# Tzq2doc/distributed_learning_simulator

Measured on AMD Instinct MI355X. Metric: FL rounds/sec (FedAvg, 100 clients, ResNet-18, CIFAR-10-shaped), higher is better.
Workload: dtype fp32; 1 GPU; fedavg_resnet18; model=ResNet18, algo=fed_avg, clients=100, local_epochs=5, global_batch=6400, per_client_batch=64, parallelism=client-dp1, backend=hip

## Files before the change

csrc/bindings.cpp:

```cpp
#include <pybind11/pybind11.h>

#include <algorithm>
#include <optional>
#include <stdexcept>
#include <string>
#include <vector>

#include "dls.h"

namespace py = pybind11;
typedef uintptr_t ptr;

template <typename T>
static T* P(ptr p) {
  return reinterpret_cast<T*>(p);
}
static hipStream_t S(ptr s) { return reinterpret_cast<hipStream_t>(s); }

extern "C" const char* dls_src_hash();

class Args {
 public:
  struct Ptr {
    uintptr_t v;
// ... 55 lines not shown
  if (!a.on()) return e;
  e.theta = a.p("theta"); e.mom = a.p("mom"); e.split = a.p("split");
  e.th_cs = a.l("th_cs"); e.sp_cs = a.l("sp_cs"); e.sp_lo = a.l("sp_lo");
  e.lr = a.p("lr"); e.active = a.p("active"); e.first = a.p("first");
  e.wd = a.f("wd"); e.momentum = a.f("momentum"); e.dampening = a.f("dampening"); e.nesterov = a.i("nesterov");
  a.finish();
  return e;
}

PYBIND11_MODULE(_dls_hip, m) {
  m.doc() = "gfx950 kernels for the MI355X-native cohort FL simulator";
  m.def("src_hash", []() { return std::string(dls_src_hash()); });
  m.def("set_native_option", [](const std::string& name, int value) {
    if (!set_native_option(name.c_str(), value)) throw std::invalid_argument("unknown native option " + name);
  });

  m.def("conv_nt", [](py::kwargs kw) {
    Args a(kw, "conv_nt");
    ConvNTParams p{};
    p.x = a.p("x"); p.w = a.p("w"); p.y = a.p("y"); p.bias = a.p("bias", 0); p.b_cs = a.l("b_cs", 0);
    p.acc = a.p("acc", 0); p.gate = a.p("gate", 0); p.x_cs = a.l("x_cs"); p.y_cs = a.l("y_cs"); p.w_cs = a.l("w_cs");
    p.B = a.i("B"); p.H = a.i("H"); p.W = a.i("W"); p.C = a.i("C"); p.OH = a.i("OH"); p.OW = a.i("OW");
    p.KH = a.i("KH"); p.KW = a.i("KW"); p.stride = a.i("stride"); p.pad = a.i("pad"); p.dil = a.i("dil");
    p.M = a.i("M"); p.N = a.i("N"); p.R = a.i("R"); p.rep = a.i("rep"); p.relu = a.i("relu", 0);
    p.b_kmajor = a.i("b_kmajor", 0); p.f32 = a.i("f32"); p.ldx = a.i("ldx", 0); p.ldy = a.i("ldy", 0);
    p.stats = a.p("stats", 0); p.stats_valid = a.p("stats_valid", 0); p.drop_seeds = a.p("drop_seeds", 0);
    p.drop_p = a.f("drop_p", 0.f); p.out_scale = a.f("out_scale", 0.f); p.wsplit = a.p("wsplit", 0);
    p.ws_cs = a.l("ws_cs", 0); p.ws_plane = a.l("ws_plane", 0); p.x_lo = a.l("x_lo", 0);
    p.yp = a.p("yp", 0); p.yp_cs = a.l("yp_cs", 0); p.yp_lo = a.l("yp_lo", 0);
    const int K = a.i("K"), variant = a.i("variant");
    const hipStream_t s = a.p("s");
    a.finish();
    if (p.stats && p.stats_valid && native_option(g_opt_halo_skip, "DLS_SKIP_INVALID", 1)) {
      p.skip_valid = p.stats_valid;
      p.skip_mul = p.OH * p.OW;
    }
    conv_nt(p, K, variant, s);
  });
  m.def("conv_dgrad", [](py::kwargs kw) {
    Args a(kw, "conv_dgrad");
    const auto dy = a.p("dy"), w = a.p("w"), acc = a.p("acc", 0), wsplit = a.p("wsplit", 0);
    const auto dx = a.p("dx"), wt_buf = a.p("wt_buf", 0), acc_mask = a.p("acc_mask", 0), s = a.p("s");
    const int K = a.i("K"), rep = a.i("rep"), B = a.i("B"), OH = a.i("OH"), OW = a.i("OW"), Co = a.i("Co");
    const int H = a.i("H"), W = a.i("W"), Ci = a.i("Ci"), KH = a.i("KH"), KW = a.i("KW"), stride = a.i("stride");
    const int pad = a.i("pad"), variant = a.i("variant"), f32 = a.i("f32"), ld_dy = a.i("ld_dy", 0);
    const int acc_compact = a.i("acc_compact", 0), wt_ready = a.i("wt_ready", 0);
    const long w_cs = a.l("w_cs"), dy_cs = a.l("dy_cs", 0), ws_cs = a.l("ws_cs", 0), ws_plane = a.l("ws_plane", 0);
    const long x_lo = a.l("x_lo", 0);
    Args b = a.sub("bnb");
    BNBwdPartials bnb{};
    if (b.on()) {
      bnb.part = b.p("part"); bnb.x = b.p("x"); bnb.xld = b.l("xld", 0); bnb.y = b.p("y", 0);
      bnb.mask = b.p("mask", 0); bnb.mean = b.p("mean"); bnb.rstd = b.p("rstd"); bnb.valid = b.p("valid", 0);
      b.finish();
    }
    a.finish();
    conv_dgrad(dy, w, dx, acc, w_cs, K, rep, B, OH, OW, Co, H, W, Ci, KH, KW, stride, pad, variant, f32, s, ld_dy,
               dy_cs, wsplit, ws_cs, ws_plane, x_lo, acc_compact, bnb.part ? &bnb : nullptr, wt_buf, acc_mask, wt_ready);
  });
  m.def("wt_planes", [](ptr wsplit, long ws_cs, long ws_plane, ptr wt, int Kw, int Co, int Ci, ptr s) {
    wt_planes(P<const bf16_t>(wsplit), ws_cs, ws_plane, P<bf16_t>(wt), Kw, Co, Ci, S(s));
  });
  m.def("conv_gl_wanted", &conv_gl_wanted);
  m.def("conv_gl_fwd", [](ptr x, ptr w, ptr y, ptr bias, long x_cs, long y_cs, long w_cs, long b_cs, int K, int rep,
                          int B, int H, int W, int C, int OH, int OW, int KH, int KW, int stride, int pad, int N,
                          int relu, ptr s) {
    conv_gl_fwd(P<const bf16_t>(x), P<const bf16_t>(w), P<bf16_t>(y), P<const bf16_t>(bias), x_cs, y_cs, w_cs, b_cs,
                K, rep, B, H, W, C, OH, OW, KH, KW, stride, pad, N, relu, S(s));
  });
  m.def("conv_weight_flip_t", [](ptr w, ptr wt, long w_cs, int Kw, int Co, int KH, int KW, int Ci, ptr s) {
    conv_weight_flip_t(P<const bf16_t>(w), P<bf16_t>(wt), w_cs, Kw, Co, KH, KW, Ci, S(s));
  });
  m.def("conv_gl_dgrad", [](ptr dy, ptr wt, ptr dx, ptr acc, int K, int rep, int B, int OH, int OW, int Co, int H, int W,
                            int Ci, int KH, int KW, int stride, int pad, ptr s) {
    conv_gl_dgrad(P<const bf16_t>(dy), P<const bf16_t>(wt), P<bf16_t>(dx), P<const bf16_t>(acc), K, rep, B, OH, OW, Co, H, W, Ci, KH, KW,
                  stride, pad, S(s));
  });
  m.def("conv_nt_num_variants", &conv_nt_num_variants);
  m.def("conv_nt_default_variant", &conv_nt_default_variant);
  m.def("conv_tn_f32_bn_bwd_ok", &conv_tn_f32_bn_bwd_ok);
  m.def("conv_tn", [](py::kwargs kw) {
    Args a(kw, "conv_tn");
    ConvTNParams p{};
    p.dy = a.p("dy"); p.x = a.p("x"); p.dw = a.p("dw");
    p.dy_cs = a.l("dy_cs"); p.x_cs = a.l("x_cs"); p.dw_cs = a.l("dw_cs");
    p.B = a.i("B"); p.H = a.i("H"); p.W = a.i("W"); p.C = a.i("C"); p.OH = a.i("OH"); p.OW = a.i("OW");
    p.KH = a.i("KH"); p.KW = a.i("KW"); p.stride = a.i("stride"); p.pad = a.i("pad");
    p.M = a.i("M"); p.Co = a.i("Co"); p.R = a.i("R"); p.splitk = 1; p.m_per_split = p.M;
    p.f32 = a.i("f32"); p.ldy = a.i("ldy", 0); p.ldx = a.i("ldx", 0);
    p.part = a.p("part", 0); p.dy_lo = a.l("dy_lo", 0); p.x_lo = a.l("x_lo", 0);
    p.sgd = sgd_arg(a.sub("sgd"));
    p.bnb_x = a.p("bnb_x", 0); p.bnb_mask = a.p("bnb_mask", 0);
    p.bnb_coef = a.p("bnb_coef", 0); p.bnb_valid = a.p("bnb_valid", 0);
    const int K = a.i("K"), variant = a.i("variant");
    const hipStream_t s = a.p("s");
    a.finish();
    conv_tn(p, K, variant, s);
  });
  m.def("conv_tn_splitk", &conv_tn_splitk, py::arg("K"), py::arg("Co"), py::arg("R"), py::arg("M"), py::arg("C"),
        py::arg("variant"), py::arg("f32"), py::arg("ldy") = 0, py::arg("ldx") = 0, py::arg("planes") = 0);
  m.def("conv_tn_pl_num_variants", &conv_tn_pl_num_variants);
  m.def("conv_tn_pl_set_variant", &conv_tn_pl_set_variant);
  m.def("conv_tn_pl_variant", &conv_tn_pl_variant);
  m.def("conv_tn_num_variants", &conv_tn_num_variants);
  m.def("conv_nt_f32_num_variants", &conv_nt_f32_num_variants);
  m.def("conv_nt_pl_num_variants", &conv_nt_pl_num_variants);
// ... 74 lines not shown
    const auto gamma = a.p("gamma"), dgamma = a.p("dgamma", 0), dbeta = a.p("dbeta", 0), ws = a.p("ws");
    const auto s = a.p("s");
    const long g_cs = a.l("g_cs"), dg_cs = a.l("dg_cs", 0);
    a.finish();
    return dense_dgrad_bn(p, gamma, g_cs, dgamma, dbeta, dg_cs, ws, s);
  });
  m.def("halo_wgrad_supported", &halo_wgrad_supported);
  m.def("halo_wgrad_part_floats", &halo_wgrad_part_floats);
  m.def("halo_wgrad", [](py::kwargs kw) {
    Args a(kw, "halo_wgrad");
    HaloWgradParams p{};
    p.sgd = sgd_arg(a.sub("sgd"));
    Args b = a.sub("bnb");
    if (b.on()) {
      p.bb_x = b.p("bb_x"); p.bb_mask = b.p("bb_mask", 0); p.bb_coef = b.p("bb_coef");
      p.bb_valid = b.p("bb_valid", 0); p.bb_dxp = b.p("bb_dxp");
      b.finish();
    }
    p.dy = a.p("dy"); p.dy_cs = a.l("dy_cs"); p.dy_lo = a.l("dy_lo", 0); p.ldy = a.i("ldy");
    p.x = a.p("x"); p.x_cs = a.l("x_cs"); p.x_lo = a.l("x_lo", 0); p.ldx = a.i("ldx");
    p.coef = a.p("coef", 0); p.relu = a.i("relu", 0); p.x_valid = a.p("x_valid", 0);
    p.valid_img = a.p("valid_img", 0); p.dw = a.p("dw"); p.dw_cs = a.l("dw_cs"); p.part = a.p("part", 0);
    p.K = a.i("K"); p.B = a.i("B"); p.H = a.i("H"); p.W = a.i("W"); p.C = a.i("C"); p.N = a.i("N");
    const int xm = a.i("xm"), dm = a.i("dm");
    const hipStream_t s = a.p("s");
    a.finish();
    return halo_wgrad(p, xm, dm, s);
  });
  m.def("conv_halo_bn_dense_supported", &conv_halo_bn_dense_supported);
  m.def("conv_halo_bn_dense_fwd", [](py::kwargs kw) {
    Args a(kw, "conv_halo_bn_dense_fwd");
    const auto x = a.p("x"), coef = a.p("coef"), valid_rows = a.p("valid_rows", 0), wsplit = a.p("wsplit");
    const auto y = a.p("y"), stats = a.p("stats", 0), stats_valid = a.p("stats_valid", 0), s = a.p("s");
    const auto ny = a.p("ny", 0), mask = a.p("mask", 0);
    const long x_cs = a.l("x_cs"), ws_cs = a.l("ws_cs"), ws_plane = a.l("ws_plane"), y_cs = a.l("y_cs");
    const long ny_cs = a.l("ny_cs", 0);
    const int ldx = a.i("ldx"), creal = a.i("creal"), relu = a.i("relu", 0), rep = a.i("rep"), ldy = a.i("ldy");
    const int K = a.i("K"), B = a.i("B"), H = a.i("H"), W = a.i("W"), C = a.i("C"), N = a.i("N"), ldny = a.i("ldny", 0);
    a.finish();
    return conv_halo_bn_dense_fwd(x, x_cs, ldx, creal, coef, relu, valid_rows, wsplit, ws_cs, ws_plane, rep, y, y_cs,
                                  ldy, K, B, H, W, C, N, stats, stats_valid, ny, ny_cs, ldny, mask, s);
  });
  m.def("bn_bwd", [](py::kwargs kw) {
    Args a(kw, "bn_bwd");
    const auto dy = a.p("dy"), x = a.p("x"), y = a.p("y", 0), mean = a.p("mean", 0);
    const auto rstd = a.p("rstd", 0), gamma = a.p("gamma", 0), valid_rows = a.p("valid_rows", 0);
    const auto dx = a.p("dx", 0), dpre = a.p("dpre", 0), dgamma = a.p("dgamma", 0);
    const auto dbeta = a.p("dbeta", 0), ws = a.p("ws"), relu_mask = a.p("relu_mask", 0), s = a.p("s");
    const auto dxp = a.p("dxp", 0), pre_part = a.p("pre_part", 0), coef_ext = a.p("coef_ext", 0);
    const long g_cs = a.l("g_cs", 0), dg_cs = a.l("dg_cs", 0);
    const int K = a.i("K"), R = a.i("R"), C = a.i("C"), relu = a.i("relu", 0), f32 = a.i("f32");
    const int ldx = a.i("ldx", 0), acc_dx = a.i("acc_dx", 0), dx_f32 = a.i("dx_f32", 1);
    const int pre_nparts = a.i("pre_nparts", 0), stage = a.i("stage", 0);
    a.finish();
    bn_bwd(dy, x, y, mean, rstd, gamma, valid_rows, g_cs, K, R, C, relu, dx, dpre, dgamma, dbeta, dg_cs, ws, relu_mask,
           f32, s, ldx, acc_dx, dxp, dx_f32, pre_part, pre_nparts, coef_ext, stage);
  });
  m.def("ln_fwd", [](ptr x, ptr gamma, ptr beta, ptr y, ptr mean, ptr rstd, long g_cs, int K, long rpc, int C,
                     float eps, int rep, int f32, ptr s, ptr yp) {
    ln_fwd(P<const void>(x), P<const void>(gamma), P<const void>(beta), P<void>(y), P<float>(mean), P<float>(rstd),
           g_cs, K, rpc, C, eps, rep, f32, S(s), P<bf16_t>(yp));
  });
  m.def("ln_bwd", [](ptr dy, ptr x, ptr mean, ptr rstd, ptr gamma, long g_cs, int K, long rpc, int C, ptr dx,
                     ptr dgamma, ptr dbeta, long dg_cs, int f32, ptr s, ptr ws) {
    ln_bwd(P<const void>(dy), P<const void>(x), P<const float>(mean), P<const float>(rstd), P<const void>(gamma), g_cs,
           K, rpc, C, P<void>(dx), P<float>(dgamma), P<float>(dbeta), dg_cs, P<float>(ws), f32, S(s));
  });
  m.def("ln_workspace_floats", &ln_workspace_floats);
  m.def("gn_shape_ok", &gn_shape_ok);
  m.def("gn_workspace_floats", &gn_workspace_floats);
  m.def("gn_fwd", [](ptr x, ptr res, ptr gamma, ptr beta, ptr y, ptr yp, ptr mean, ptr rstd, ptr valid, long g_cs,
                     int rep, int K, int B, int HW, int C, int G, float eps, int relu, int f32, ptr s) {
    gn_fwd(P<const void>(x), P<const void>(res), P<const void>(gamma), P<const void>(beta), P<void>(y), P<bf16_t>(yp),
           P<float>(mean), P<float>(rstd), P<const int>(valid), g_cs, rep, K, B, HW, C, G, eps, relu, f32, S(s));
  });
  m.def("gn_bwd", [](ptr dy, ptr x, ptr y, ptr mean, ptr rstd, ptr gamma, ptr valid, long g_cs, int rep, int K, int B,
                     int HW, int C, int G, int relu, ptr dx, ptr dres, ptr dgamma, ptr dbeta, long dg_cs, ptr ws,
                     int f32, ptr s) {
    gn_bwd(P<const void>(dy), P<const void>(x), P<const void>(y), P<const float>(mean), P<const float>(rstd),
           P<const void>(gamma), P<const int>(valid), g_cs, rep, K, B, HW, C, G, relu, P<void>(dx), P<void>(dres),
           P<float>(dgamma), P<float>(dbeta), dg_cs, P<float>(ws), f32, S(s));
  });
  m.def("col_sum_workspace_floats", &col_sum_workspace_floats);
  m.def("col_sum", [](ptr x, ptr out, long out_cs, int K, long rows, int C, int f32, ptr s, ptr ws) {
    col_sum(P<const void>(x), P<float>(out), out_cs, K, rows, C, f32, S(s), P<float>(ws));
  });

  m.def("pool_fwd", [](ptr x, ptr y, ptr idx, int K, int B, int H, int W, int C, int OH, int OW, int k, int stride,
                       int pad, int mode, int f32, ptr s) {
    pool_fwd(P<const void>(x), P<void>(y), P<int>(idx), K, B, H, W, C, OH, OW, k, stride, pad, mode, f32, S(s));
  });
  m.def("pool_bwd", [](ptr dy, ptr idx, ptr dx, int K, int B, int H, int W, int C, int OH, int OW, int k, int stride,
                       int pad, int mode, int f32, ptr s) {
    pool_bwd(P<const void>(dy), P<const int>(idx), P<void>(dx), K, B, H, W, C, OH, OW, k, stride, pad, mode, f32, S(s));
  });
  m.def("gap_fwd", [](ptr x, ptr y, int KB, int HW, int C, int f32, ptr s) {
    gap_fwd(P<const void>(x), P<void>(y), KB, HW, C, f32, S(s));
  });
  m.def("gap_bwd", [](ptr dy, ptr dx, int KB, int HW, int C, int f32, ptr s) {
    gap_bwd(P<const void>(dy), P<void>(dx), KB, HW, C, f32, S(s));
  });
  m.def("ce_fwd_bwd", [](ptr logits, ptr labels, ptr valid, ptr loss, ptr correct, ptr dlogits, int K, int B, int NC,
                         int f32, ptr s, ptr rowbuf) {
    ce_fwd_bwd(P<const void>(logits), P<const int>(labels), P<const int>(valid), P<float>(loss), P<float>(correct),
               P<void>(dlogits), K, B, NC, f32, S(s), P<float>(rowbuf));
  });
  m.def("relu_bwd", [](ptr dy, ptr y, ptr dx, long n, int f32, ptr s) {
    relu_bwd(P<const void>(dy), P<const void>(y), P<void>(dx), n, f32, S(s));
  });

// ... 227 lines not shown
```

csrc/conv_f32.hip:

```cpp
#include "dls.h"
#include "gemm_common.h"
#include "epilogue_f32.h"

#include <numeric>

namespace {

template <int V>
struct FV {
  float v[V];
};

template <int V>
__device__ __forceinline__ void fzero(FV<V>& f) {
#pragma unroll
  for (int i = 0; i < V; ++i) f.v[i] = 0.f;
}

template <int V>
__device__ __forceinline__ void fload(FV<V>& f, const float* p) {
  load_vec<V>(p, f.v);
}

template <int V>
// ... 231 lines not shown
#pragma unroll
      for (int j = 0; j < TN; ++j) {
        if constexpr (!BKM) {
          const int r = wn0 + j * 32 + (lane & 31);
          const int off = (buf * B_ROWS + r) * B_COLS + swz<BK>(r, ks * 16 + 8 * h);
          bh[j] = *reinterpret_cast<const bf16x8*>(Bs + off);
          bl[j] = *reinterpret_cast<const bf16x8*>(Bs + B_PLANE + off);
        } else {
          const int col = wn0 + j * 32 + 16 * (g & 1) + 4 * pp;
          const int o0 = (buf * B_ROWS + ks * 16 + 8 * h + q) * B_COLS + col;
          const int o1 = o0 + 4 * B_COLS;
          bh[j] = tr_frag(Bs + o0, Bs + o1);
          bl[j] = tr_frag(Bs + B_PLANE + o0, Bs + B_PLANE + o1);
        }
      }
#pragma unroll
      for (int i = 0; i < TM; ++i)
#pragma unroll
        for (int j = 0; j < TN; ++j) {
          acc[i][j] = __builtin_amdgcn_mfma_f32_32x32x16_bf16(al[i], bh[j], acc[i][j], 0, 0, 0);
          acc[i][j] = __builtin_amdgcn_mfma_f32_32x32x16_bf16(ah[i], bl[j], acc[i][j], 0, 0, 0);
          acc[i][j] = __builtin_amdgcn_mfma_f32_32x32x16_bf16(ah[i], bh[j], acc[i][j], 0, 0, 0);
        }
    }
  };

  if constexpr (NBUF == 1) {
    load();
    store(0);
    __syncthreads();
    for (int kt = 0; kt < nk; ++kt) {
      if (kt + 1 < nk) load();
      compute(0);
      if (kt + 1 < nk) {
        __syncthreads();
        store(0);
        __syncthreads();
      }
    }
  } else {
    load();
    store(0);
    __syncthreads();
    int buf = 0;
    for (int kt = 0; kt < nk; ++kt) {
      if (kt + 1 < nk) load();
      compute(buf);
      if (kt + 1 < nk) store(buf ^ 1);
      __syncthreads();
      buf ^= 1;
    }
  }

  nt_f32_epilogue<TM, TN, WM * WN, -1, false>(p, acc, smem, client, m0, n0, wm0, wn0, wid, lane);
}

template <int BM, int BN, int BK, int WM, int WN, int NBUF, int VSET, int MINW = 1>
bool launch_nt_f32_cfg(const ConvNTParams& p, int K, int va, int vb, bool bkm, hipStream_t s) {
  const int grid = K * cdiv(p.M, BM) * cdiv(p.N, BN);
  if (p.wsplit && va == 8 && vb == 8) {
    if (bkm)
      hipLaunchKernelGGL((conv_nt_f32_kernel<BM, BN, BK, WM, WN, 8, 8, true, NBUF, MINW, true>), dim3(grid),
                         dim3(WM * WN * 64), 0, s, p);
    else
      hipLaunchKernelGGL((conv_nt_f32_kernel<BM, BN, BK, WM, WN, 8, 8, false, NBUF, MINW, true>), dim3(grid),
                         dim3(WM * WN * 64), 0, s, p);
    return true;
  }
#define NTF_CASE(A, B)                                                                                       \
  if (va == A && vb == B) {                                                                                  \
    if (bkm)                                                                                                 \
      hipLaunchKernelGGL((conv_nt_f32_kernel<BM, BN, BK, WM, WN, A, B, true, NBUF, MINW>), dim3(grid),             \
                         dim3(WM * WN * 64), 0, s, p);                                                       \
    else                                                                                                     \
      hipLaunchKernelGGL((conv_nt_f32_kernel<BM, BN, BK, WM, WN, A, B, false, NBUF, MINW>), dim3(grid),            \
                         dim3(WM * WN * 64), 0, s, p);                                                       \
    return true;                                                                                             \
  }
  NTF_CASE(8, 8)
  if constexpr (VSET >= 1) { NTF_CASE(4, 4) NTF_CASE(8, 4) NTF_CASE(4, 8) }
  if constexpr (VSET >= 2) { NTF_CASE(8, 1) NTF_CASE(4, 1) NTF_CASE(1, 8) NTF_CASE(1, 4) NTF_CASE(1, 1) }
#undef NTF_CASE
  return false;
}

bool launch_nt_f32_variant(int v, const ConvNTParams& p, int K, int va, int vb, bool bkm, hipStream_t s) {
  switch (v) {
    case 0: return launch_nt_f32_cfg<128, 128, 32, 2, 2, 2, 1>(p, K, va, vb, bkm, s);
    case 1: return launch_nt_f32_cfg<128, 128, 32, 2, 2, 1, 0>(p, K, va, vb, bkm, s);
    case 2: return launch_nt_f32_cfg<256, 128, 32, 4, 2, 1, 0>(p, K, va, vb, bkm, s);
    case 3: return launch_nt_f32_cfg<64, 64, 32, 2, 2, 2, 2>(p, K, va, vb, bkm, s);
    case 4: return launch_nt_f32_cfg<128, 64, 32, 4, 1, 2, 1>(p, K, va, vb, bkm, s);
    case 5: return launch_nt_f32_cfg<128, 128, 64, 2, 2, 1, 0>(p, K, va, vb, bkm, s);
    case 6: return launch_nt_f32_cfg<256, 64, 32, 4, 1, 1, 0>(p, K, va, vb, bkm, s);
    case 7: return launch_nt_f32_cfg<64, 64, 32, 2, 2, 1, 1>(p, K, va, vb, bkm, s);
    case 8: return launch_nt_f32_cfg<128, 128, 32, 2, 2, 1, 0, 3>(p, K, va, vb, bkm, s);
    case 9: return launch_nt_f32_cfg<256, 64, 32, 4, 1, 1, 0, 3>(p, K, va, vb, bkm, s);
    case 10: return launch_nt_f32_cfg<256, 32, 32, 4, 1, 1, 1>(p, K, va, vb, bkm, s);
    default: return false;
  }
}

int vw(int c) { return (c % 8 == 0) ? 8 : (c % 4 == 0) ? 4 : 1; }


template <int BMc, int BNr, int BKT, int WM, int WN, int VA, int VB, int NBUF, bool BNB = false>
__global__ void __launch_bounds__(WM* WN * 64) conv_tn_f32_kernel(ConvTNParams p) {
// ... 317 lines not shown
  (void)K;
  const TnTile t = kTnF32Tiles[variant];
  const long tiles = (long)32 * cdiv(Co, t.bm) * cdiv(R, t.bn);
  splitk = 1;
  const int target = 1024;
  if (tiles < target) {
    splitk = (int)((target + tiles - 1) / tiles);
    splitk = min(splitk, max(1, M / (4 * TN_BKT_MAX)));
  }
  mps = cdiv(M, splitk);
  mps = ((mps + TN_BKT_MAX - 1) / TN_BKT_MAX) * TN_BKT_MAX;
  splitk = cdiv(M, mps);
}

}

int conv_nt_f32_num_variants() { return 11; }

void conv_nt_f32(const ConvNTParams& p, int K, int variant, hipStream_t s) {
  if (p.x_lo != 0) {
    if (conv_nt_pl_variant() < 0 && conv_halo(p, K, s)) return;
    if (!conv_nt_pl(p, K, conv_nt_pl_variant(), s)) {
      fprintf(stderr, "conv_nt_f32: pre-split operands in an unsupported shape (C %d, ldx %d, N %d, R %d)\n", p.C,
              p.ldx, p.N, p.R);
      abort();
    }
    return;
  }
  const bool bkm = p.b_kmajor != 0;
  const long xb = (long)p.B * p.H * p.W * p.ldx * 4;
  const long wb = (bkm ? (long)p.C * p.wKH * p.wKW * p.N : (long)p.N * p.R) * 4;
  if (p.dil != 1) {
    fprintf(stderr, "conv_nt_f32: input dilation is not supported\n");
    abort();
  }
  if (xb >= (long)OOB_OFF || wb >= (long)OOB_OFF || (p.wsplit && (p.ws_plane + wb / 4) * 2 >= (long)OOB_OFF)) {
    fprintf(stderr, "conv_nt_f32: per-client operand window over 2 GiB (x %ld B, w %ld B)\n", xb, wb);
    abort();
  }
  const int va = vw(std::gcd(p.C, p.ldx));
  int vb = bkm ? vw(p.N) : vw(p.R);
  if (variant < 0) {
    variant = p.N <= 64 ? 9 : 1;
    if (p.N <= 32) variant = 10;
    if (p.N > 64 && p.KH * p.KW == 1) variant = 8;
  }
  const bool v88 = va == 8 && vb == 8;
  const bool v84 = (va == 8 || va == 4) && (vb == 8 || vb == 4);
  if (!v88) {
    if (!v84 && variant != 3) variant = 3;
    if (v84 && !(variant == 0 || variant == 3 || variant == 4 || variant == 7 || variant == 10))
      variant = p.N <= 64 ? 4 : 0;
  }
  if (!launch_nt_f32_variant(variant, p, K, va, vb, bkm, s)) fprintf(stderr, "conv_nt_f32: bad variant %d\n", variant);
  if (p.yp) {
    if (p.yp_cs != 2 * p.y_cs || p.yp_lo != p.y_cs || p.ldy != p.N || p.out_s != 1) {
      fprintf(stderr, "conv_nt_f32: output planes need contiguous per-client rows\n");
      abort();
    }
    split_rows(reinterpret_cast<const float*>(p.y), p.yp, K, (long)p.M * p.N, p.y_cs, s);
  }
}

int conv_tn_f32_num_variants() { return kTnF32Variants; }

void conv_tn_f32(ConvTNParams p, int K, int variant, hipStream_t s) {
  if (p.sgd.theta && p.dy_lo == 0) {
    fprintf(stderr, "conv_tn_f32: the SGD epilogue needs pre-split operands\n");
    abort();
  }
  if (p.dy_lo != 0) {
    if (!conv_tn_pl(p, K, variant, s)) {
      fprintf(stderr, "conv_tn_f32: pre-split operands in an unsupported shape (C %d, Co %d)\n", p.C, p.Co);
      abort();
    }
    return;
  }
  const long dyb = (long)p.M * (p.ldy ? p.ldy : p.Co) * 4, xb = (long)p.B * p.H * p.W * (p.ldx ? p.ldx : p.C) * 4;
  if (dyb >= (long)OOB_OFF || xb >= (long)OOB_OFF) {
    fprintf(stderr, "conv_tn_f32: per-client operand window over 2 GiB (dy %ld B, x %ld B)\n", dyb, xb);
    abort();
  }
  const int va = vw(std::gcd(p.Co, p.ldy));
  const int vb = vw(std::gcd(p.C, p.ldx));
  variant = resolve_tn_f32_variant(variant, K, p.Co, p.R, va, vb);
  if (p.bnb_coef && !(p.bnb_x && p.ldy == p.Co && p.dy_cs == (long)p.M * p.Co && va == 8 && vb == 8 &&
                      tn_f32_bnb_variant(variant))) {
    fprintf(stderr, "conv_tn_f32: the BN-backward loader does not serve this launch (Co %d, C %d, variant %d)\n",
            p.Co, p.C, variant);
    abort();
  }
  tn_f32_split(K, p.Co, p.R, p.M, variant, p.splitk, p.m_per_split);
  const TnTile t = kTnF32Tiles[variant];
  const long tiles = (long)K * cdiv(p.Co, t.bm) * cdiv(p.R, t.bn);
  const int grid = (int)(tiles * p.splitk);
  if (!launch_tn_f32_variant(variant, p, va, vb, grid, s)) fprintf(stderr, "conv_tn_f32: bad variant %d\n", variant);
  if (p.splitk > 1 && p.part != nullptr) tn_fold(p.part, p.dw, p.dw_cs, K, p.splitk, (long)p.Co * p.R, s);
}

bool conv_tn_f32_bn_bwd_ok(int K, int Co, int R, int gco, int gc, int variant) {
  const int va = vw(gco), vb = vw(gc);
  return va == 8 && vb == 8 && tn_f32_bnb_variant(resolve_tn_f32_variant(variant, K, Co, R, va, vb));
}

int conv_tn_f32_splitk(int K, int Co, int R, int M, int gco, int gc, int variant) {
  int splitk, mps;
// ... 5 lines not shown
```

csrc/conv_nt.hip:

```cpp
#include "dls.h"
#include "gemm_common.h"

#include <numeric>

namespace {

template <int BM, int BN, int BK, int WM, int WN, int VA, int VB, bool BKM, int DEPTH>
__global__ void __launch_bounds__(WM* WN * 64) conv_nt_kernel(ConvNTParams p) {
  constexpr int T = WM * WN * 64;
  constexpr int TM = BM / (WM * 32);
  constexpr int TN = BN / (WN * 32);
  constexpr int LDA = BK + 8;
  constexpr int KCA = BK / VA, RPA = T / KCA, PA = BM / RPA;
  constexpr int KCB = BK / VB, RPB = T / KCB, PB = BN / RPB;
  constexpr int CCB = BN / VB, RPK = T / CCB, PK = BK / RPK;
  constexpr int LDBK = BN + 32;
  constexpr int NB = BKM ? PK : PB;
  static_assert(PA >= 1 && NB >= 1, "tile too small for thread count");
  static_assert(TM >= 1 && TN >= 1, "wave tile");
  constexpr int NBUF = DEPTH == 0 ? 1 : 2;
  constexpr int B_ROWS = BKM ? BK : BN, B_COLS = BKM ? LDBK : LDA;
  constexpr int A_BYTES = NBUF * BM * LDA * 2, B_BYTES = NBUF * B_ROWS * B_COLS * 2;
  constexpr int SW = TN * 32 + 8;
  constexpr int EPI_BYTES = WM * WN * 32 * SW * 2;
// ... 335 lines not shown
  if (p.wKH == 0) {
    p.pad_w = p.pad;
    p.wKH = p.KH;
    p.wKW = p.KW;
    p.kh_off = p.KH - 1;
    p.kw_off = p.KW - 1;
    p.kh_step = p.kw_step = 1;
  }
  if (p.out_s == 0) p.out_s = 1;
  if (p.ldx == 0) p.ldx = p.C;
  if (p.ldy == 0) p.ldy = p.N;
  p.fd_ohw = make_fastdiv((uint32_t)(p.OH * p.OW));
  p.fd_ow = make_fastdiv((uint32_t)p.OW);
  p.fd_kwc = make_fastdiv((uint32_t)(p.KW * p.C));
  p.fd_c = make_fastdiv((uint32_t)p.C);
  if (p.f32) {
    conv_nt_f32(p, K, variant, s);
    return;
  }
  if (p.stats) {
    fprintf(stderr, "conv_nt: epilogue statistics need the fp32 kernels\n");
    abort();
  }
  const bool bkm = p.b_kmajor != 0;
  int va = vec_width(std::gcd(p.C, p.ldx));
  int vb = bkm ? vec_width(p.N) : vec_width(p.R);
  if (va == 1 && vb == 4) vb = 1;
  if (variant < 0) {
    variant = conv_nt_default_variant(p.M, p.N, p.R, p.b_kmajor);
    (void)K;
  }
  const bool w84 = (va == 8 || va == 4) && (vb == 8 || vb == 4);
  if (w84 && !(va == 8 && vb == 8) && !(variant == 0 || variant == 10 || variant == 13 || variant == 6 ||
                                        variant == 7 || variant == 18)) {
    variant = (p.N <= 64) ? 13 : (bkm ? 10 : 0);
  } else if (!w84 && !(variant == 6 || variant == 7 || variant == 18)) {
    variant = (p.N <= 64) ? 7 : 6;
  }
  if (!launch_variant(variant, p, K, va, vb, bkm, s)) fprintf(stderr, "conv_nt: bad variant %d\n", variant);
}

void wt_planes(const bf16_t* wsplit, long ws_cs, long ws_plane, bf16_t* wt, int Kw, int Co, int Ci, hipStream_t s) {
  hipLaunchKernelGGL(wt_planes_kernel, dim3(Kw * 2 * 9, Co / 32, Ci / 32), dim3(256), 0, s, wsplit, ws_cs, ws_plane, wt,
                     Co, Ci);
}

void conv_dgrad(const bf16_t* dy, const bf16_t* w, bf16_t* dx, const bf16_t* acc, long w_cs, int K, int rep, int B, int OH, int OW,
                int Co, int H, int W, int Ci, int KH, int KW, int stride, int pad, int variant, int f32, hipStream_t s,
                int ld_dy, long dy_cs, const bf16_t* wsplit, long ws_cs, long ws_plane, long x_lo, int acc_compact,
                const BNBwdPartials* bnb, bf16_t* wt_buf, const uint8_t* acc_mask, int wt_ready) {
  ConvNTParams p{};
  p.acc_mask = acc_mask;
  if (bnb) {
    if (!f32 || stride != 1 || Ci % 4 != 0 || (bnb->mask && Ci % 8 != 0) || (bnb->xld && bnb->xld % 4 != 0)) {
      fprintf(stderr, "conv_dgrad: BN-backward partials need an fp32 stride-1 dgrad with Ci %% 4 == 0\n");
      abort();
    }
    p.bnb = bnb->part;
    p.bnb_x = bnb->x;
    p.bnb_xld = bnb->xld ? bnb->xld : Ci;
    p.bnb_y = bnb->y;
    p.bnb_mask = bnb->mask;
    p.bnb_mean = bnb->mean;
    p.bnb_rstd = bnb->rstd;
    p.bnb_valid = bnb->valid;
    if (stride == 1 && bnb->valid && native_option(g_opt_halo_skip, "DLS_SKIP_INVALID", 1)) {
      p.skip_valid = bnb->valid;
      p.skip_mul = 1;
    }
  }
  p.x_lo = x_lo;
  p.wsplit = wsplit;
  p.ws_cs = ws_cs;
  p.ws_plane = ws_plane;
  p.f32 = f32;
  p.ldx = ld_dy;
  p.x = dy;
  p.w = w;
  p.y = dx;
  p.bias = nullptr;
  p.acc = acc;
  p.x_cs = dy_cs ? dy_cs : (long)B * OH * OW * (ld_dy ? ld_dy : Co);
  p.y_cs = (long)B * H * W * Ci;
  p.w_cs = w_cs;
  p.b_cs = 0;
  p.B = B;
  p.H = OH;
  p.W = OW;
  p.C = Co;
  p.N = Ci;
  p.rep = rep;
  p.relu = 0;
  p.b_kmajor = 1;
  p.wKH = KH;
  p.wKW = KW;
  p.dil = 1;
  p.stride = 1;
  if (stride == 1) {
    p.OH = H;
    p.OW = W;
    p.KH = KH;
    p.KW = KW;
    p.pad = KH - 1 - pad;
    p.pad_w = KW - 1 - pad;
    p.kh_off = KH - 1;
    p.kw_off = KW - 1;
    p.kh_step = p.kw_step = 1;
    p.out_s = 1;
    p.M = B * H * W;
    p.R = KH * KW * Co;
    if (variant < 0 && !f32 && Ci <= 64 && vec_width(Ci) == 8 && vec_width(Co) == 8) variant = 14;
    if (wt_buf && f32 && x_lo != 0 && wsplit && KH == 3 && KW == 3 && pad == 1 && Co % 32 == 0 && Ci % 32 == 0) {
      const int Kw = K / rep;
      if (!wt_ready)
        hipLaunchKernelGGL(wt_planes_kernel, dim3(Kw * 2 * 9, Co / 32, Ci / 32), dim3(256), 0, s, wsplit, ws_cs,
                           ws_plane, wt_buf, Co, Ci);
      p.b_kmajor = 0;
      p.wsplit = wt_buf;
      p.ws_cs = 2L * 9 * Ci * Co;
      p.ws_plane = 9L * Ci * Co;
      p.w = wt_buf;
      p.w_cs = p.ws_cs;
    }
    conv_nt(p, K, variant, s);
    return;
  }
  for (int ph = 0; ph < stride; ++ph) {
    const int Hc = (H - ph + stride - 1) / stride;
    if (Hc <= 0) continue;
    const int kh0 = (ph + pad) % stride;
    const int nkh = kh0 < KH ? (KH - kh0 + stride - 1) / stride : 0;
    const int dh = (ph + pad - kh0) / stride;
    for (int pw = 0; pw < stride; ++pw) {
      const int Wc = (W - pw + stride - 1) / stride;
      if (Wc <= 0) continue;
      const int kw0 = (pw + pad) % stride;
      const int nkw = kw0 < KW ? (KW - kw0 + stride - 1) / stride : 0;
      const int dw = (pw + pad - kw0) / stride;
      ConvNTParams q = p;
      q.OH = Hc;
      q.OW = Wc;
      q.M = B * Hc * Wc;
      if (acc_compact) {
        q.acc = (ph == 0 && pw == 0) ? acc : nullptr;
        q.acc_compact = 1;
        q.acc_cs = (long)B * Hc * Wc * Ci;
      }
      q.out_s = stride;
      q.out_ph = ph;
      q.out_pw = pw;
      q.out_H = H;
      q.out_W = W;
      if (nkh == 0 || nkw == 0) {
        q.KH = q.KW = 1;
        q.R = 0;
        q.pad = q.pad_w = 0;
        q.kh_off = q.kw_off = 0;
        q.kh_step = q.kw_step = 1;
      } else {
        q.KH = nkh;
        q.KW = nkw;
        q.pad = nkh - 1 - dh;
        q.pad_w = nkw - 1 - dw;
        q.kh_off = kh0 + stride * (nkh - 1);
        q.kw_off = kw0 + stride * (nkw - 1);
        q.kh_step = q.kw_step = stride;
        q.R = nkh * nkw * Co;
      }
      conv_nt(q, K, variant, s);
    }
  }
}
```

csrc/conv_pl.hip:

```cpp
#include "dls.h"
#include "epilogue_f32.h"
#include "sgd_epi.h"
#include "gemm_common.h"

#include <algorithm>
#include <cstdlib>

namespace {

constexpr int PK = 32;

typedef __attribute__((address_space(3))) void lds_void;

__device__ __forceinline__ void dma16(__amdgpu_buffer_rsrc_t r, unsigned char* lds, uint32_t off) {
  __builtin_amdgcn_raw_ptr_buffer_load_lds(r, (lds_void*)lds, 16, off, 0, 0, 0);
}

template <int N>
__device__ __forceinline__ void wait_vm() {
  static_assert(N >= 0 && N < 64, "vmcnt range");
  __builtin_amdgcn_s_waitcnt((N & 15) | ((N >> 4) << 14) | (7 << 4) | (15 << 8));
}

template <int BM, int BN, int WM, int WN, bool BKM, int NST, int MINW, bool ILV, int PKT, bool PIX = false>
// ... 193 lines not shown
      for (int i = 0; i < TM; ++i) {
        if (PIX && !on[i]) continue;
#pragma unroll
        for (int j = 0; j < TN; ++j) {
          acc[i][j] = __builtin_amdgcn_mfma_f32_32x32x16_bf16(al[i], bh[j], acc[i][j], 0, 0, 0);
          acc[i][j] = __builtin_amdgcn_mfma_f32_32x32x16_bf16(ah[i], bl[j], acc[i][j], 0, 0, 0);
          acc[i][j] = __builtin_amdgcn_mfma_f32_32x32x16_bf16(ah[i], bh[j], acc[i][j], 0, 0, 0);
          if constexpr (ILV) {
            static_assert(!ILV || !PIX, "the interleaved DMAs must issue with every triple");
            const int tri = (ks * TM + i) * TN + j;
#pragma unroll
            for (int n = 0; n < G; ++n)
              if ((n * NTRI) / G == tri) {
                piece(n, nb);
                __builtin_amdgcn_sched_group_barrier(0x008, 3, 0);
                __builtin_amdgcn_sched_group_barrier(0x020, 1, 0);
              }
          }
        }
      }
    }
    if constexpr (PIX) {
      c_kc += PKT;
      if (c_kc == p.C) {
        c_kc = 0;
        if (++c_kw > tb.w1) {
          c_kw = tb.w0;
          ++c_kh;
        }
      }
    }
  };

  const int nk = PIX ? (tb.h1 - tb.h0 + 1) * (tb.w1 - tb.w0 + 1) * (p.C / PKT) : p.R / PKT;
#pragma unroll
  for (int st = 0; st < NST - 1; ++st) {
    prep(st < nk);
#pragma unroll
    for (int n = 0; n < G; ++n) piece(n, st);
  }
  for (int kt = 0; kt < nk; ++kt) {
    wait_vm<G*(NST - 2)>();
    __builtin_amdgcn_s_barrier();
    const int nb = (kt + NST - 1) % NST;
    prep(kt + NST - 1 < nk);
    if constexpr (!ILV) {
#pragma unroll
      for (int n = 0; n < G; ++n) piece(n, nb);
    }
    compute(kt % NST, nb);
  }
  wait_vm<0>();

  nt_f32_epilogue<TM, TN, NW, -1, true, PIX>(p, acc, smem, client, m0, n0, wm0, wn0, wid, lane);
}

template <int BM, int BN, int WM, int WN, int NST, bool ILV = false, int PKT = 32, int MINW = 1, bool PIX = false>
void launch_pl(const ConvNTParams& p, int K, bool bkm, hipStream_t s) {
  const int grid = K * cdiv(p.M, BM) * cdiv(p.N, BN);
  if (bkm)
    hipLaunchKernelGGL((conv_nt_pl_kernel<BM, BN, WM, WN, true, NST, MINW, ILV, PKT, PIX>), dim3(grid),
                       dim3(WM * WN * 64), 0, s, p);
  else
    hipLaunchKernelGGL((conv_nt_pl_kernel<BM, BN, WM, WN, false, NST, MINW, ILV, PKT, PIX>), dim3(grid),
                       dim3(WM * WN * 64), 0, s, p);
}

}

static int g_pl_variant = -1;
int conv_nt_pl_variant() { return g_pl_variant; }
void conv_nt_pl_set_variant(int v) { g_pl_variant = v; }

int conv_nt_pl_num_variants() { return 8; }

bool conv_nt_pl_supported(const ConvNTParams& p) {
  return p.x_lo != 0 && p.wsplit != nullptr && p.dil == 1 && p.C % PK == 0 && p.ldx % 8 == 0 &&
         p.N % 8 == 0 && (p.R == p.KH * p.KW * p.C || p.R == 0);
}

static int pl_min_wg() {
  return native_option(g_opt_pl_min_wg, "DLS_PL_MIN_WG", 192);
}

int conv_nt_pl_default_variant(const ConvNTParams& p, int K) {
  if (p.N <= 64) return 2;
  if (p.N >= 512) return (long)K * cdiv(p.M, 256) * cdiv(p.N, 256) < pl_min_wg() ? 1 : 3;
  if (p.M >= (1 << 17)) {
    if (p.N >= 256) return 3;
    if (p.KH * p.KW > 1) return 4;
  }
  return 1;
}

static bool pix_ok(const ConvNTParams& p, int variant) {
  return native_option(g_opt_conv_pix, "DLS_CONV_PIX", 1) != 0 && variant == 3 && p.stride == 1 &&
         p.OH * p.OW <= 64 && p.KH * p.KW > 1 && (p.pad > 0 || p.pad_w > 0) && p.out_s <= 1 && !p.acc_compact &&
         !(p.drop_p > 0.f) && p.M == p.B * p.OH * p.OW;
}

bool conv_nt_pl(const ConvNTParams& p0, int K, int variant, hipStream_t s) {
  if (!conv_nt_pl_supported(p0)) return false;
  const long ab = (p0.x_lo + (long)p0.B * p0.H * p0.W * p0.ldx) * 2;
  const long wb = (p0.ws_plane + (p0.b_kmajor ? (long)p0.C * p0.wKH * p0.wKW * p0.N : (long)p0.N * p0.R)) * 2;
  if (ab >= (long)OOB_OFF || wb >= (long)OOB_OFF) return false;
  if (variant < 0) variant = conv_nt_pl_default_variant(p0, K);
  const bool bkm = p0.b_kmajor != 0;
// ... 438 lines not shown
```

csrc/dls.h:

```cpp
#pragma once
#include <hip/hip_runtime.h>
#include <stdint.h>

typedef uint16_t bf16_t;

constexpr int kOptUnset = -1000000;
extern int g_opt_attn_mfma, g_opt_conv_gl, g_opt_pl_min_wg;
extern int g_opt_halo_wgrad_unroll;
extern int g_opt_halo_skip;
extern int g_opt_conv_pix;
int native_option(int& slot, const char* env, int dflt);
bool set_native_option(const char* name, int value);

struct FastDiv {
  uint32_t d, mul, shift;
};

static inline FastDiv make_fastdiv(uint32_t d) {
  FastDiv f;
  f.d = d;
  uint32_t s = 0;
  while ((1u << s) < d) ++s;
  f.shift = s;
  f.mul = (uint32_t)((((uint64_t)1 << 32) * (((uint64_t)1 << s) - d)) / d + 1);
  return f;
}

__device__ __forceinline__ uint32_t fdiv(uint32_t n, const FastDiv& f) {
  return (__umulhi(n, f.mul) + n) >> f.shift;
}

struct ConvNTParams {
  const bf16_t* x;
  const bf16_t* w;
  bf16_t* y;
  const bf16_t* bias;
  const bf16_t* acc;
  long acc_cs;
  int acc_compact;
  const uint8_t* acc_mask;
  const bf16_t* gate;
  long x_cs, y_cs, w_cs, b_cs;
  int B, H, W, C;
  int OH, OW, KH, KW, stride, pad, dil;
  int pad_w;
  int M, N, R;
  int rep;
  int relu;
  int b_kmajor;
  int wKH, wKW, kh_off, kh_step, kw_off, kw_step;
  int out_s, out_ph, out_pw, out_H, out_W;
  FastDiv fd_ohw, fd_ow, fd_kwc, fd_c;
  int f32;
  int ldx, ldy;
  float* stats;
  const int* stats_valid;
  const uint32_t* drop_seeds;
  float drop_p;
  float out_scale;
  const bf16_t* wsplit;
  long ws_cs, ws_plane;
  long x_lo;
  float* bnb;
  const float* bnb_x;
  long bnb_xld;
  const float* bnb_y;
  const uint8_t* bnb_mask;
  const float* bnb_mean;
  const float* bnb_rstd;
  const int* bnb_valid;
  const float* bn_x;
  long bn_x_cs;
  const float* bn_coef;
  int bn_relu;
  const int* bn_valid;
  bf16_t* bn_yp;
  uint8_t* bn_mask;
  int bn_c;
  float* bn_y;
  long bn_y_cs;
  int bn_ldy;
  const int* skip_valid;
  int skip_mul;
  bf16_t* yp;
  long yp_cs, yp_lo;
  int pix;
  FastDiv fd_pb;
};

struct BNBwdPartials {
  float* part;
  const float* x;
  long xld;
  const float* y;
  const uint8_t* mask;
  const float* mean;
  const float* rstd;
  const int* valid;
};

struct DenseWgradParams {
  const float* dy;
  long dy_cs;
  int ldy;
  const float* y;
  long y_cs;
  float* dw;
  long dw_cs;
  float* part;
  int K, B, H, W, C, N, nchunks, G;
  const float* bn_sc;
  int ldy_x;
  const int* valid_rows;
};

struct DenseDgradParams {
  const float* dy;
  long dy_cs;
  int ldy;
  const float* w;
  long w_cs;
  int rep;
  const float* x;
  float* dx;
  long x_cs;
  int ldx;
  const uint8_t* mask;
  const float* y;
  const float* bn_sc;
  const float* mean;
  const float* rstd;
  const int* valid_rows;
  const float* coef;
  float* part;
  int K, B, H, W, C, N, G, nchunks;
};

struct SgdEpi {
  float* theta;
  float* mom;
  bf16_t* split;
  long th_cs, sp_cs, sp_lo;
  const float* lr;
  const uint8_t* active;
  const uint8_t* first;
  float wd, momentum, dampening;
  int nesterov;
};

struct HaloWgradParams {
  const void* dy;
// ... 108 lines not shown
bool conv_halo_bn_fwd(const float* x, long x_cs, const float* coef, int relu, const int* valid_rows,
                      const bf16_t* wsplit, long ws_cs, long ws_plane, int rep, float* y, long y_cs, int K, int B,
                      int H, int W, int C, int N, float* stats, const int* stats_valid, hipStream_t s,
                      bf16_t* yp = nullptr, uint8_t* mask = nullptr);
bool conv_halo_bn_dense_supported(int B, int H, int W, int C, int N);
bool conv_halo_bn_dense_fwd(const float* x, long x_cs, int ldx, int creal, const float* coef, int relu,
                            const int* valid_rows, const bf16_t* wsplit, long ws_cs, long ws_plane, int rep, float* y,
                            long y_cs, int ldy, int K, int B, int H, int W, int C, int N, float* stats,
                            const int* stats_valid, float* ny, long ny_cs, int ldny, uint8_t* mask, hipStream_t s);
bool dense_dgrad_supported(int B, int H, int W, int C, int N);
long dense_dgrad_ws_floats(int K, int B, int H, int C);
bool dense_dgrad_bn(DenseDgradParams p, const float* gamma, long g_cs, float* dgamma, float* dbeta, long dg_cs,
                    float* ws, hipStream_t s);
void bn_bwd_coef_parts(const float* part, int nparts, const float* gamma, long g_cs, const int* valid_rows,
                       const float* mean, const float* rstd, int K, int R, int C, float* coef, float* dgamma,
                       float* dbeta, long dg_cs, hipStream_t s);
bool dense_wgrad_supported(int B, int H, int W, int C, int N);
long dense_wgrad_part_floats(int K, int B, int H, int W, int C);
bool dense_wgrad(const float* dy, long dy_cs, int ldy, const float* y, long y_cs, float* dw, long dw_cs, float* part,
                 int K, int B, int H, int W, int C, int N, hipStream_t s, const float* bn_sc = nullptr,
                 int ldy_x = 0, const int* valid_rows = nullptr);
void conv_halo_set_mode(int m);
void conv_halo_set_variant(int v);
bool conv_tn_pl_supported(const ConvTNParams& p);
bool conv_tn_pl(ConvTNParams p, int K, int variant, hipStream_t s);
int conv_tn_pl_num_variants();
int conv_tn_pl_variant();
void conv_tn_pl_set_variant(int v);
int conv_tn_pl_splitk(int K, int Co, int R, int M, int variant);
void tn_fold(const float* part, float* dw, long dw_cs, int K, int splitk, long CoR, hipStream_t s,
             const SgdEpi* sgd = nullptr);
int conv_tn_f32_num_variants();
int conv_tn_f32_splitk(int K, int Co, int R, int M, int gco, int gc, int variant);
bool conv_tn_f32_bn_bwd_ok(int K, int Co, int R, int gco, int gc, int variant);

long bn_workspace_floats(int K, long R, int C);
void bn_fwd(const void* x, const void* gamma, const void* beta, const void* res, void* y, float* mean, float* rstd,
            const int* valid_rows, long g_cs, int K, int R, int C, int relu, float eps, int rep, float* ws,
            uint8_t* relu_mask, int f32, hipStream_t s,
            int ldx = 0, const float* pre_part = nullptr,
            int pre_nparts = 0, bf16_t* yp = nullptr,
            int y_f32 = 1, float* coef_out = nullptr, int apply = 1,
            const float* res_coef = nullptr,
            int res_relu = 0);
void bn_bwd(const void* dy, const void* x, const void* y, const float* mean, const float* rstd, const void* gamma,
            const int* valid_rows, long g_cs, int K, int R, int C, int relu, void* dx, void* dpre, float* dgamma,
            float* dbeta, long dg_cs, float* ws, const uint8_t* relu_mask, int f32,
            hipStream_t s, int ldx = 0,
            int acc_dx = 0, bf16_t* dxp = nullptr,
            int dx_f32 = 1,
            const float* pre_part = nullptr,
            int pre_nparts = 0,
            float* coef_ext = nullptr,
            int stage = 0);
void ln_fwd(const void* x, const void* gamma, const void* beta, void* y, float* mean, float* rstd, long g_cs, int K,
            long rows_per_client, int C, float eps, int rep, int f32, hipStream_t s,
            bf16_t* yp = nullptr);
void ln_bwd(const void* dy, const void* x, const float* mean, const float* rstd, const void* gamma, long g_cs, int K,
            long rows_per_client, int C, void* dx, float* dgamma, float* dbeta, long dg_cs, float* ws, int f32,
            hipStream_t s);
long col_sum_workspace_floats(int K, long rows, int C);
long ln_workspace_floats(int K, long rows_per_client, int C);
bool gn_shape_ok(int HW, int C, int G);
long gn_workspace_floats(int K, int B, int C);
void gn_fwd(const void* x, const void* res, const void* gamma, const void* beta, void* y, bf16_t* yp, float* mean,
            float* rstd, const int* valid, long g_cs, int rep, int K, int B, int HW, int C, int G, float eps, int relu,
            int f32, hipStream_t s);
void gn_bwd(const void* dy, const void* x, const void* y, const float* mean, const float* rstd, const void* gamma,
            const int* valid, long g_cs, int rep, int K, int B, int HW, int C, int G, int relu, void* dx, void* dres,
            float* dgamma, float* dbeta, long dg_cs, float* ws, int f32, hipStream_t s);
void col_sum(const void* x, float* out, long out_cs, int K, long rows, int C, int f32, hipStream_t s,
             float* ws = nullptr);

void pool_fwd(const void* x, void* y, int* idx, int K, int B, int H, int W, int C, int OH, int OW, int k, int stride,
              int pad, int mode, int f32, hipStream_t s);
void pool_bwd(const void* dy, const int* idx, void* dx, int K, int B, int H, int W, int C, int OH, int OW, int k,
              int stride, int pad, int mode, int f32, hipStream_t s);
void gap_fwd(const void* x, void* y, int KB, int HW, int C, int f32, hipStream_t s);
void gap_bwd(const void* dy, void* dx, int KB, int HW, int C, int f32, hipStream_t s);
void ce_fwd_bwd(const void* logits, const int* labels, const int* valid, float* loss, float* correct, void* dlogits,
                int K, int B, int NC, int f32, hipStream_t s, float* rowbuf = nullptr);
void relu_bwd(const void* dy, const void* y, void* dx, long n, int f32, hipStream_t s);

void quant_pack(const float* x, long ld, const int* seg, const int64_t* seg_off, const int64_t* seg_numel,
                const uint8_t* bits, const float* lo, const float* scale, const int64_t* seg_byte_off,
                const int64_t* row_off, int K, int nseg, long P, int stochastic, const uint32_t* seeds, uint8_t* out,
                hipStream_t s);
void quant_unpack(const uint8_t* codes, const int* seg, const int64_t* seg_off, const int64_t* seg_numel,
                  const uint8_t* bits, const float* lo, const float* scale, const int64_t* seg_byte_off,
                  const int64_t* row_off, int K, int nseg, long P, float* out, long ld, hipStream_t s);
void quant_unpack_acc(const uint8_t* codes, const int* seg, const int64_t* seg_off, const int64_t* seg_numel,
                      const uint8_t* bits, const float* lo, const float* scale, const int64_t* seg_byte_off,
                      const int64_t* row_off, int K, int nseg, long P, const double* w, double* acc, hipStream_t s);

#define TOPK_CHUNK 4096
void topk_pack(const float* delta, long ld_d, float* u, long ld_u, int ef, const uint32_t* vbits, uint32_t* hist,
               uint32_t* state, uint32_t* cnt, uint32_t* excl, int* idx, float* val, int K, long P, int k,
               hipStream_t s);
void topk_decode(const int* idx, const float* val, float* out, long ld, int K, long P, int k, hipStream_t s);
void topk_accumulate(const int* idx, const float* val, const double* w, double* acc, int K, long P, int k,
                     hipStream_t s);

#define ROTSIGN_BLOCK 4096
void rotsign_pack(const float* delta, long ld_d, float* err, long ld_e, const uint32_t* vbits, const uint32_t* seeds,
                  uint8_t* bits, float* scale, int K, long P, int mse, hipStream_t s);
void rotsign_unpack(const uint8_t* bits, const float* scale, const uint32_t* vbits, const uint32_t* seeds, float* out,
                    long ld, int K, long P, hipStream_t s);
// ... 120 lines not shown
```

csrc/epilogue_f32.h:

```cpp
#pragma once
#include "dls.h"
#include "gemm_common.h"

template <int TM, int TN, int NW, int PF = -1, bool YP = true, bool PIX = false>
__device__ __forceinline__ void nt_f32_epilogue(const ConvNTParams& p, f32x16 (&acc)[TM][TN], unsigned char* smem,
                                                int client, int m0, int n0, int wm0, int wn0, int wid, int lane) {
  constexpr int SW = TN * 32 + 4;
  float* __restrict__ y = reinterpret_cast<float*>(p.y) + (long)client * p.y_cs;
  const float* accp =
      p.acc ? reinterpret_cast<const float*>(p.acc) + (long)client * (p.acc_compact ? p.acc_cs : p.y_cs) : nullptr;
  const float* gatep = p.gate ? reinterpret_cast<const float*>(p.gate) + (long)client * p.y_cs : nullptr;
  const uint8_t* amask = (accp && p.acc_mask) ? p.acc_mask + (long)client * (p.y_cs >> 3) : nullptr;
  bf16_t* ypl = (YP && p.yp) ? p.yp + (long)client * p.yp_cs : nullptr;
  auto store_pl4 = [&](long off, const float4& v) {
    uint32_t h0, l0, h1, l1;
    split_pair(v.x, v.y, h0, l0);
    split_pair(v.z, v.w, h1, l1);
    *reinterpret_cast<uint2*>(ypl + off) = make_uint2(h0, h1);
    *reinterpret_cast<uint2*>(ypl + p.yp_lo + off) = make_uint2(l0, l1);
  };
  auto store_pl1 = [&](long off, float v) {
    uint32_t h, l;
    split_pair(v, 0.f, h, l);
    ypl[off] = (bf16_t)(h & 0xffffu);
    ypl[p.yp_lo + off] = (bf16_t)(l & 0xffffu);
  };
  auto abits = [&](long row, int n, bool ok) -> uint32_t {
    return amask ? (ok ? (uint32_t)(amask[row * (p.N >> 3) + (n >> 3)] >> (n & 4)) : 0u) : 0xFu;
  };
  const float* bias = p.bias ? reinterpret_cast<const float*>(p.bias) + (long)(client / p.rep) * p.b_cs : nullptr;
  const bool drop = p.drop_p > 0.f && p.drop_seeds != nullptr;
  const uint32_t dseed = drop ? p.drop_seeds[client] : 0u;
  const float oscale = (p.out_scale != 0.f ? p.out_scale : 1.f) * (drop ? 1.f / (1.f - p.drop_p) : 1.f);
  float bvals[TN];
#pragma unroll
  for (int j = 0; j < TN; ++j) {
    const int n = n0 + wn0 + j * 32 + (lane & 31);
    bvals[j] = (bias && n < p.N) ? bias[n] : 0.f;
  }
  float* slab = reinterpret_cast<float*>(smem) + wid * 32 * SW;
  const bool vec_ok = (p.N % 4) == 0 && (p.ldy % 4) == 0 && ((uintptr_t)y & 15) == 0;
  const int stat_rows = p.stats ? (p.stats_valid ? min(p.M, p.stats_valid[client] * p.OH * p.OW) : p.M) : 0;
  static_assert(TN == 1 || TN == 2 || TN == 4 || TN == 8, "column quads per row must divide the wave");
  constexpr int Q = TN * 8;
  const bool bnb = p.bnb != nullptr;
  const int bnb_rows = bnb ? (p.bnb_valid ? min(p.M, p.bnb_valid[client]) : p.M) : 0;
  float4 bmu = make_float4(0.f, 0.f, 0.f, 0.f), brs = bmu;
  {
    const int n = n0 + wn0 + (lane % Q) * 4;
    if (bnb && n < p.N) {
      bmu = *reinterpret_cast<const float4*>(p.bnb_mean + (long)client * p.N + n);
      brs = *reinterpret_cast<const float4*>(p.bnb_rstd + (long)client * p.N + n);
    }
  }
  constexpr int QPL = 4 * TN;
  const float* bx_base = bnb ? p.bnb_x + (long)client * p.M * p.bnb_xld : nullptr;
  const unsigned char* bm_base = (bnb && p.bnb_mask) ? p.bnb_mask + (long)client * p.M * (p.N >> 3) : nullptr;
  const float* by_base = (bnb && p.bnb_y) ? p.bnb_y + (long)client * p.y_cs : nullptr;
  auto ld4 = [](const float* base, long off, bool ok) {
    const float4 v = *reinterpret_cast<const float4*>(ok ? base + off : base);
    return ok ? v : make_float4(0.f, 0.f, 0.f, 0.f);
  };
  auto row_of = [&](int m) -> long {
    if constexpr (PIX) {
      const uint32_t px = fdiv((uint32_t)m, p.fd_pb);
      return (long)((uint32_t)m - px * (uint32_t)p.B) * (p.OH * p.OW) + px;
    }
    if (p.out_s > 1) {
      const uint32_t b = fdiv(m, p.fd_ohw);
      const uint32_t rem = m - b * p.OH * p.OW;
      const uint32_t oh = fdiv(rem, p.fd_ow);
      const uint32_t ow = rem - oh * p.OW;
      return ((long)b * p.out_H + oh * p.out_s + p.out_ph) * p.out_W + ow * p.out_s + p.out_pw;
    }
    return m;
  };
  auto vrow = [&](int m) -> long {
    if constexpr (PIX) return row_of(m);
    return m;
  };
  __syncthreads();
#pragma unroll
  for (int i = 0; i < TM; ++i) {
    const int g0 = m0 + wm0 + i * 32;
    if (p.stats && g0 < p.M) {
      float* part = p.stats + ((long)client * ((p.M + 31) / 32) + g0 / 32) * 2 * p.N;
#pragma unroll
      for (int j = 0; j < TN; ++j) {
        float s0 = 0.f, s1 = 0.f;
#pragma unroll
        for (int e = 0; e < 16; ++e) {
          const int m = g0 + (e & 3) + 8 * (e >> 2) + 4 * (lane >> 5);
          float v = acc[i][j][e] + bvals[j];
          if (p.relu) v = fmaxf(v, 0.f);
          if (vrow(m) < stat_rows) {
            s0 += v;
            s1 = fmaf(v, v, s1);
          }
        }
        s0 += __shfl_xor(s0, 32, 64);
        s1 += __shfl_xor(s1, 32, 64);
        const int n = n0 + wn0 + j * 32 + (lane & 31);
        if (lane < 32 && n < p.N) {
          part[n] = s0;
          part[p.N + n] = s1;
        }
      }
    }
    float4 bs0 = make_float4(0.f, 0.f, 0.f, 0.f), bs1 = bs0;
    if constexpr (PF > 0) {
      const int cc = (lane % Q) * 4, n = n0 + wn0 + cc;
      constexpr int NS = PF > 0 ? PF : 1;
      float4 av[NS], xv[NS];
      uint32_t mv[NS], amv[NS];
      auto issue = [&](int t) {
        const int m = m0 + wm0 + i * 32 + lane / Q + t * (64 / Q);
        const bool ok = n < p.N && m < p.M;
        const long row = row_of(m);
        if (accp) av[t % NS] = ld4(accp, (p.acc_compact ? (long)m : row) * p.ldy + n, ok);
        if (amask) amv[t % NS] = abits(row, n, ok);
        if (bnb) {
          const bool okb = ok && vrow(m) < bnb_rows;
          xv[t % NS] = ld4(bx_base, row * p.bnb_xld + n, okb);
          if (bm_base) {
            const uint32_t mb = *(okb ? bm_base + vrow(m) * (p.N >> 3) + (n >> 3) : bm_base);
            mv[t % NS] = okb ? (mb >> (n & 4)) : 0u;
          } else if (by_base) {
            const float4 yv = ld4(by_base, row * p.ldy + n, okb);
            mv[t % NS] = (yv.x > 0.f ? 1u : 0u) | (yv.y > 0.f ? 2u : 0u) | (yv.z > 0.f ? 4u : 0u) | (yv.w > 0.f ? 8u : 0u);
          } else {
            mv[t % NS] = okb ? 0xFu : 0u;
          }
        }
      };
      if (vec_ok) {
#pragma unroll
        for (int t = 0; t < PF && t < QPL; ++t) issue(t);
      }
#pragma unroll
      for (int j = 0; j < TN; ++j) {
#pragma unroll
        for (int e = 0; e < 16; ++e) {
          float v = acc[i][j][e] + bvals[j];
          if (p.relu) v = fmaxf(v, 0.f);
          v *= oscale;
          if (drop) {
            const int rr = (e & 3) + 8 * (e >> 2) + 4 * (lane >> 5);
            if (!drop_keep(dseed, m0 + wm0 + i * 32 + rr, p.N, n0 + wn0 + j * 32 + (lane & 31), p.drop_p)) v = 0.f;
          }
          slab[((e & 3) + 8 * (e >> 2) + 4 * (lane >> 5)) * SW + j * 32 + (lane & 31)] = v;
        }
      }
      __builtin_amdgcn_s_waitcnt(0xC07F);
      __builtin_amdgcn_s_barrier();
      if (vec_ok) {
#pragma unroll
        for (int t = 0; t < QPL; ++t) {
          const int r = lane / Q + t * (64 / Q);
          const int m = m0 + wm0 + i * 32 + r;
          const long row = row_of(m);
          float4 v = *reinterpret_cast<const float4*>(slab + r * SW + cc);
          if (gatep) {
            const float4 gv = ld4(gatep, row * p.ldy + n, n < p.N && m < p.M);
            v.x = gv.x > 0.f ? v.x : 0.f;
            v.y = gv.y > 0.f ? v.y : 0.f;
            v.z = gv.z > 0.f ? v.z : 0.f;
            v.w = gv.w > 0.f ? v.w : 0.f;
          }
          if (accp) {
            const uint32_t ab = amask ? amv[t % NS] : 0xFu;
            v.x += (ab & 1u) ? av[t % NS].x : 0.f;
            v.y += (ab & 2u) ? av[t % NS].y : 0.f;
            v.z += (ab & 4u) ? av[t % NS].z : 0.f;
            v.w += (ab & 8u) ? av[t % NS].w : 0.f;
          }
          if (n < p.N && m < p.M) {
            *reinterpret_cast<float4*>(y + row * p.ldy + n) = v;
            if (YP && ypl) store_pl4(row * p.ldy + n, v);
// ... 22 lines not shown
          const long arow = p.acc_compact ? (long)m : row;
          for (int t2 = 0; t2 < 4 && nn + t2 < p.N; ++t2) {
            float o = slab[r * SW + c4 + t2];
            if (gatep && !(gatep[row * p.ldy + nn + t2] > 0.f)) o = 0.f;
            if (accp && ((abits(row, nn + t2, true) >> ((nn + t2) & 3)) & 1u)) o += accp[arow * p.ldy + nn + t2];
            y[row * p.ldy + nn + t2] = o;
            if (YP && ypl) store_pl1(row * p.ldy + nn + t2, o);
          }
        }
      }
    } else {
#pragma unroll
      for (int j = 0; j < TN; ++j) {
#pragma unroll
        for (int e = 0; e < 16; ++e) {
          float v = acc[i][j][e] + bvals[j];
          if (p.relu) v = fmaxf(v, 0.f);
          v *= oscale;
          if (drop) {
            const int rr = (e & 3) + 8 * (e >> 2) + 4 * (lane >> 5);
            if (!drop_keep(dseed, m0 + wm0 + i * 32 + rr, p.N, n0 + wn0 + j * 32 + (lane & 31), p.drop_p)) v = 0.f;
          }
          slab[((e & 3) + 8 * (e >> 2) + 4 * (lane >> 5)) * SW + j * 32 + (lane & 31)] = v;
        }
      }
      __syncthreads();
      for (int qd = lane; qd < 32 * TN * 8; qd += 64) {
        const int r = qd / (TN * 8), cc = (qd % (TN * 8)) * 4;
        const int m = m0 + wm0 + i * 32 + r, n = n0 + wn0 + cc;
        if (m >= p.M || n >= p.N) continue;
        const long row = row_of(m);
        float* dst = y + row * p.ldy + n;
        const float* src = slab + r * SW + cc;
        const long arow = p.acc_compact ? (long)m : row;
        if (vec_ok && n + 4 <= p.N) {
          float4 v = *reinterpret_cast<const float4*>(src);
          if (gatep) {
            const float4 gv = *reinterpret_cast<const float4*>(gatep + row * p.ldy + n);
            v.x = gv.x > 0.f ? v.x : 0.f;
            v.y = gv.y > 0.f ? v.y : 0.f;
            v.z = gv.z > 0.f ? v.z : 0.f;
            v.w = gv.w > 0.f ? v.w : 0.f;
          }
          if (accp) {
            const float4 av = *reinterpret_cast<const float4*>(accp + arow * p.ldy + n);
            const uint32_t ab = abits(row, n, true);
            v.x += (ab & 1u) ? av.x : 0.f;
            v.y += (ab & 2u) ? av.y : 0.f;
            v.z += (ab & 4u) ? av.z : 0.f;
            v.w += (ab & 8u) ? av.w : 0.f;
          }
          *reinterpret_cast<float4*>(dst) = v;
          if (YP && ypl) store_pl4(row * p.ldy + n, v);
          if (bnb && vrow(m) < bnb_rows) {
            const float4 xv =
                *reinterpret_cast<const float4*>(p.bnb_x + ((long)client * p.M + row) * p.bnb_xld + n);
            uint32_t mb = 0xFu;
            if (p.bnb_mask) {
              mb = p.bnb_mask[((long)client * p.M + vrow(m)) * (p.N >> 3) + (n >> 3)] >> (n & 4);
            } else if (p.bnb_y) {
              const float4 yv = *reinterpret_cast<const float4*>(p.bnb_y + (long)client * p.y_cs + row * p.ldy + n);
              mb = (yv.x > 0.f ? 1u : 0u) | (yv.y > 0.f ? 2u : 0u) | (yv.z > 0.f ? 4u : 0u) | (yv.w > 0.f ? 8u : 0u);
            }
            const float g0 = (mb & 1u) ? v.x : 0.f, g1 = (mb & 2u) ? v.y : 0.f;
            const float g2 = (mb & 4u) ? v.z : 0.f, g3 = (mb & 8u) ? v.w : 0.f;
            bs0.x += g0;
            bs0.y += g1;
            bs0.z += g2;
            bs0.w += g3;
            bs1.x = fmaf(g0, (xv.x - bmu.x) * brs.x, bs1.x);
            bs1.y = fmaf(g1, (xv.y - bmu.y) * brs.y, bs1.y);
            bs1.z = fmaf(g2, (xv.z - bmu.z) * brs.z, bs1.z);
            bs1.w = fmaf(g3, (xv.w - bmu.w) * brs.w, bs1.w);
          }
        } else {
          for (int t2 = 0; t2 < 4 && n + t2 < p.N; ++t2) {
            float o = src[t2];
            if (gatep && !(gatep[row * p.ldy + n + t2] > 0.f)) o = 0.f;
            if (accp && ((abits(row, n + t2, true) >> ((n + t2) & 3)) & 1u)) o += accp[arow * p.ldy + n + t2];
            dst[t2] = o;
            if (YP && ypl) store_pl1(row * p.ldy + n + t2, o);
          }
        }
      }
    }
    if (bnb) {
#pragma unroll
      for (int off = Q; off < 64; off <<= 1) {
        bs0.x += __shfl_xor(bs0.x, off, 64);
        bs0.y += __shfl_xor(bs0.y, off, 64);
        bs0.z += __shfl_xor(bs0.z, off, 64);
        bs0.w += __shfl_xor(bs0.w, off, 64);
        bs1.x += __shfl_xor(bs1.x, off, 64);
        bs1.y += __shfl_xor(bs1.y, off, 64);
        bs1.z += __shfl_xor(bs1.z, off, 64);
        bs1.w += __shfl_xor(bs1.w, off, 64);
      }
      const int g0 = m0 + wm0 + i * 32, n = n0 + wn0 + lane * 4;
      if (lane < Q && g0 < p.M && n < p.N) {
        float* part = p.bnb + ((long)client * ((p.M + 31) / 32) + g0 / 32) * 2 * p.N;
        *reinterpret_cast<float4*>(part + n) = bs0;
        *reinterpret_cast<float4*>(part + p.N + n) = bs1;
      }
    }
    __syncthreads();
  }
}
```

csrc/norm.hip:

```cpp
#include "common.h"
#include <algorithm>
#include <numeric>

#include "dls.h"

namespace {

constexpr int ROWS_PER_BLOCK = 512;

static int rows_per_block(long R, int K) {
  const long want = std::min<long>(64, (2048 + K - 1) / K);
  const long bpc = std::max(1L, std::min(want, std::max(1L, R / 64)));
  return (int)std::min<long>(ROWS_PER_BLOCK, (R + bpc - 1) / bpc);
}

struct BNCoefArgs {
  const void* gamma;
  const void* beta;
  const float* mean_in;
  const float* rstd_in;
  float* mean_out;
  float* rstd_out;
  float* coef;
  float* dgamma;
// ... 340 lines not shown
#pragma unroll
    for (int j = 0; j < V; ++j) {
      sc[j] = coef[2 * ((long)k * C + c0 + j)];
      sh[j] = coef[2 * ((long)k * C + c0 + j) + 1];
      rsc[j] = res_coef ? res_coef[2 * ((long)k * C + c0 + j)] : 0.f;
      rsh[j] = res_coef ? res_coef[2 * ((long)k * C + c0 + j) + 1] : 0.f;
    }
    for (int r = r0 + rl; r < r1; r += RT) {
      const long off = base + (long)r * C + c0;
      float out[V];
      if (r < nvalid) {
        float v[V];
        const long offx = base_x + (long)r * ldx + c0;
        load_vec<V>(x + offx, v);
#pragma unroll
        for (int j = 0; j < V; ++j) out[j] = fmaf(v[j], sc[j], sh[j]);
        if (res) {
          float rv[V];
          load_vec<V>(res + offx, rv);
          if (res_coef && res_relu) {
#pragma unroll
            for (int j = 0; j < V; ++j) out[j] += fmaxf(fmaf(rv[j], rsc[j], rsh[j]), 0.f);
          } else if (res_coef) {
#pragma unroll
            for (int j = 0; j < V; ++j) out[j] += fmaf(rv[j], rsc[j], rsh[j]);
          } else {
#pragma unroll
            for (int j = 0; j < V; ++j) out[j] += rv[j];
          }
        }
        if (relu) {
#pragma unroll
          for (int j = 0; j < V; ++j) out[j] = fmaxf(out[j], 0.f);
        }
      } else {
#pragma unroll
        for (int j = 0; j < V; ++j) out[j] = 0.f;
      }
      if (rmask) {
        uint32_t m = 0;
#pragma unroll
        for (int j = 0; j < V; ++j) m |= (rt<T>(out[j]) > 0.f ? 1u : 0u) << j;
        rmask[((long)k * R + r) * (C / 8) + c0 / 8] = (uint8_t)m;
      }
      if (y_f32) store_vec<V>(y + off, out);
      if (yp) {
        bf16_t* hp = yp + (long)k * R * C + off;
        store_planes<V>(hp, hp + (long)R * C, out);
      }
    }
  }
}

template <typename T, int V>
__global__ void __launch_bounds__(256) bn_bwd_apply_kernel(const T* __restrict__ dy, const T* __restrict__ x,
                                                           const T* __restrict__ y,
                                                           const int* __restrict__ valid_rows,
                                                           const float* __restrict__ coef, int R, int C, int relu,
                                                           T* __restrict__ dx, T* __restrict__ dpre,
                                                           int rpb, const uint8_t* __restrict__ rmask, int ldx,
                                                           int acc_dx, bf16_t* __restrict__ dxp, int dx_f32) {
  const int k = blockIdx.y;
  const int CT = C / V;
  const int nvalid = valid_rows ? min(valid_rows[k], R) : R;
  const int r0 = blockIdx.x * rpb, r1 = min(R, r0 + rpb);
  const long base = (long)k * R * C, base_x = (long)k * R * ldx;
  for (int cg = 0; cg < CT; cg += 256) {
    const int ctn = min(256, CT - cg);
    const int RT = 256 / ctn;
    const int cc = threadIdx.x % ctn, rl = threadIdx.x / ctn;
    if (rl >= RT) continue;
    const int c0 = (cg + cc) * V;
    float ca[V], cd[V], ce[V];
#pragma unroll
    for (int j = 0; j < V; ++j) {
      const long q = 3 * ((long)k * C + c0 + j);
      ca[j] = coef[q];
      cd[j] = coef[q + 1];
      ce[j] = coef[q + 2];
    }
    for (int r = r0 + rl; r < r1; r += RT) {
      const long off = base + (long)r * C + c0;
      const long offx = base_x + (long)r * ldx + c0;
      float o[V], gp[V];
      if (r < nvalid) {
        float vdy[V], vx[V];
        load_vec<V>(dy + off, vdy);
        load_vec<V>(x + offx, vx);
        if (rmask) {
          const uint32_t mbits = rmask[((long)k * R + r) * (C / 8) + c0 / 8];
#pragma unroll
          for (int j = 0; j < V; ++j) vdy[j] = ((mbits >> j) & 1u) ? vdy[j] : 0.f;
        } else if (relu) {
          float vy[V];
          load_vec<V>(y + off, vy);
#pragma unroll
          for (int j = 0; j < V; ++j) vdy[j] = vy[j] > 0.f ? vdy[j] : 0.f;
        }
#pragma unroll
        for (int j = 0; j < V; ++j) {
          gp[j] = vdy[j];
          o[j] = fmaf(ca[j], vdy[j], fmaf(ce[j], vx[j], cd[j]));
        }
      } else {
#pragma unroll
        for (int j = 0; j < V; ++j) o[j] = gp[j] = 0.f;
      }
      if (acc_dx) {
        float prev[V];
        load_vec<V>(dx + offx, prev);
#pragma unroll
        for (int j = 0; j < V; ++j) o[j] += prev[j];
      }
      if (dx_f32) store_vec<V>(dx + offx, o);
      if (dxp) {
        bf16_t* hp = dxp + (long)k * R * C + off;
        store_planes<V>(hp, hp + (long)R * C, o);
      }
      if (dpre) store_vec<V>(dpre + off, gp);
    }
  }
}

int vw(int C) { return (C % 8 == 0) ? 8 : (C % 4 == 0) ? 4 : 1; }

template <typename T>
__global__ void __launch_bounds__(256) ln_fwd_kernel(const T* __restrict__ x, const T* __restrict__ gamma,
                                                     const T* __restrict__ beta, T* __restrict__ y,
                                                     float* __restrict__ mean, float* __restrict__ rstd, long g_cs,
                                                     long nrows, long rpc, int C, float eps, int rep,
                                                     bf16_t* __restrict__ yp) {
  const long row = (long)blockIdx.x * 4 + (threadIdx.x >> 6);
  const int lane = threadIdx.x & 63;
  if (row >= nrows) return;
  const int k = (int)(row / rpc);
  const T* xr = x + row * C;
  float s = 0.f, sq = 0.f;
  for (int c = lane; c < C; c += 64) s += ldf(xr + c);
  const float mu = wave_sum(s) / C;
  for (int c = lane; c < C; c += 64) {
    const float d = ldf(xr + c) - mu;
    sq += d * d;
  }
  const float rs = rsqrtf(wave_sum(sq) / C + eps);
  const T* g = gamma + (long)(k / rep) * g_cs;
  const T* b = beta + (long)(k / rep) * g_cs;
  bf16_t* hp = yp ? yp + (row + (long)k * rpc) * C : nullptr;
  for (int c = lane; c < C; c += 64) {
    const float o = (ldf(xr + c) - mu) * rs * ldf(g + c) + ldf(b + c);
    stf(y + row * C + c, o);
    if (hp) {
      bf16_t h, l;
      split2(rt<T>(o), h, l);
      hp[c] = h;
      hp[rpc * C + c] = l;
    }
  }
  if (lane == 0) {
    mean[row] = mu;
    rstd[row] = rs;
  }
}

template <int NC2>
__global__ void __launch_bounds__(256) ln_fwd_pairs_kernel(const float* __restrict__ x,
                                                           const float* __restrict__ gamma,
                                                           const float* __restrict__ beta, float* __restrict__ y,
                                                           float* __restrict__ mean, float* __restrict__ rstd,
                                                           long g_cs, long nrows, long rpc, int C, float eps, int rep,
                                                           bf16_t* __restrict__ yp) {
  const long row = (long)blockIdx.x * 4 + (threadIdx.x >> 6);
  const int lane = threadIdx.x & 63;
// ... 108 lines not shown
      const int c = lane + 64 * i;
      if (c < C) {
        if (part) {
          float* pw = part + ((long)k * gridDim.x * 4 + wave) * 2 * C;
          pw[c] = dg[i];
          pw[C + c] = db[i];
        } else {
          atomicAdd(&dgamma[(long)k * dg_cs + c], dg[i]);
          atomicAdd(&dbeta[(long)k * dg_cs + c], db[i]);
        }
      }
    }
  }
}

__global__ void __launch_bounds__(256) part_sum_kernel(const float* __restrict__ part, int nparts, int W, int C,
                                                       float* __restrict__ out0, float* __restrict__ out1, long out_cs) {
  const int k = blockIdx.y, c = blockIdx.x * 256 + threadIdx.x;
  if (c >= C) return;
  const float* p = part + (long)k * nparts * W;
  float a = 0.f, b = 0.f;
  for (int i = 0; i < nparts; ++i) {
    a += p[(long)i * W + c];
    if (out1) b += p[(long)i * W + C + c];
  }
  out0[(long)k * out_cs + c] = a;
  if (out1) out1[(long)k * out_cs + c] = b;
}

}

#define DISPATCH_V(V, ...)          \
  if (V == 8) {                     \
    constexpr int VV = 8;           \
    __VA_ARGS__;                    \
  } else if (V == 4) {              \
    constexpr int VV = 4;           \
    __VA_ARGS__;                    \
  } else {                          \
    constexpr int VV = 1;           \
    __VA_ARGS__;                    \
  }
#define DISPATCH_T(F32, ...)        \
  if (F32) {                        \
    typedef float TT;               \
    __VA_ARGS__;                    \
  } else {                          \
    typedef bf16_t TT;              \
    __VA_ARGS__;                    \
  }
#define CP(p) static_cast<const TT*>(p)
#define MP(p) static_cast<TT*>(p)

static long bn_fold_offset(int K, long R, int C) {
  const long parts = (R + rows_per_block(R, K) - 1) / rows_per_block(R, K);
  return ((long)K * 3 * C + (long)K * parts * 2 * C + 1) & ~1L;
}

long bn_workspace_floats(int K, long R, int C) {
  const long nfold = cdiv((int)cdiv((int)R, 32), FOLD);
  return bn_fold_offset(K, R, C) + (long)K * nfold * 2 * C * 2;
}

void bn_fwd(const void* x, const void* gamma, const void* beta, const void* res, void* y, float* mean, float* rstd,
            const int* valid_rows, long g_cs, int K, int R, int C, int relu, float eps, int rep, float* ws,
            uint8_t* rmask, int f32, hipStream_t s, int ldx, const float* pre_part,
            int pre_nparts, bf16_t* yp, int y_f32, float* coef_out, int apply, const float* res_coef,
            int res_relu) {
  if (ldx == 0) ldx = C;
  float* coef = coef_out ? coef_out : ws;
  const float* part = pre_part ? pre_part : ws + (long)3 * C * K;
  const int rpb = rows_per_block(R, K);
  dim3 grid(cdiv(R, rpb), K);
  const int nparts = pre_part ? pre_nparts : (int)grid.x;
  const int V = vw(std::gcd(C, ldx));
  BNCoefArgs ca{gamma, beta, nullptr, nullptr, mean, rstd, coef, nullptr, nullptr, 0L, g_cs, eps, rep, 0};
  if (V != 8) rmask = nullptr;
  DISPATCH_T(f32, {
    if (!pre_part) {
      DISPATCH_V(V, hipLaunchKernelGGL((chan_reduce_kernel<TT, VV, 0>), grid, dim3(256), 0, s, CP(x), nullptr, nullptr,
                                       nullptr, nullptr, valid_rows, R, C, 0, ws + (long)3 * C * K, (long)2 * C, rpb,
                                       nullptr, ca, ldx, ldx));
    }
    if (pre_part && nparts > FOLD && nparts <= cdiv(R, 32)) {
      const int nfold = cdiv(nparts, FOLD);
      double* folds = reinterpret_cast<double*>(ws + bn_fold_offset(K, R, C));
      hipLaunchKernelGGL(part_fold_kernel, dim3(nfold, K), dim3(256), 0, s, pre_part, nparts, 2 * C, folds, nfold);
      launch_coef<TT, double>(dim3(cdiv(C, 32), K), s, (const double*)folds, nfold, CP(gamma), CP(beta), valid_rows,
                              (const float*)nullptr, (const float*)nullptr, mean, rstd, coef, (float*)nullptr,
                              (float*)nullptr, 0L, g_cs, K, R, C, eps, rep, 0, 0, 0L);
    } else {
      launch_coef<TT, float>(dim3(cdiv(C, 32), K), s, part, nparts, CP(gamma), CP(beta), valid_rows,
                             (const float*)nullptr, (const float*)nullptr, mean, rstd, coef, (float*)nullptr,
                             (float*)nullptr, 0L, g_cs, K, R, C, eps, rep, 0, 0, 0L);
    }
    if (apply) {
      DISPATCH_V(V, hipLaunchKernelGGL((bn_apply_kernel<TT, VV>), grid, dim3(256), 0, s, CP(x), CP(res), MP(y),
                                       valid_rows, coef, R, C, relu, rpb, rmask, ldx, f32 ? yp : nullptr,
                                       f32 ? y_f32 : 1, res_coef, res_relu));
    }
  });
}

void bn_apply_only(const float* x, const float* coef, const int* valid_rows, int K, int R, int C, int relu,
                   bf16_t* yp, uint8_t* rmask, hipStream_t s, float* y) {
  const int rpb = rows_per_block(R, K);
  dim3 grid(cdiv(R, rpb), K);
  if (C % 8 == 0) {
    hipLaunchKernelGGL((bn_apply_kernel<float, 8>), grid, dim3(256), 0, s, x, (const float*)nullptr, y,
                       valid_rows, coef, R, C, relu, rpb, rmask, C, yp, y ? 1 : 0, (const float*)nullptr, 0);
  } else {
    hipLaunchKernelGGL((bn_apply_kernel<float, 1>), grid, dim3(256), 0, s, x, (const float*)nullptr, y,
                       valid_rows, coef, R, C, relu, rpb, (uint8_t*)nullptr, C, yp, y ? 1 : 0, (const float*)nullptr,
                       0);
  }
}

void bn_bwd(const void* dy, const void* x, const void* y, const float* mean, const float* rstd, const void* gamma,
            const int* valid_rows, long g_cs, int K, int R, int C, int relu, void* dx, void* dpre, float* dgamma,
            float* dbeta, long dg_cs, float* ws, const uint8_t* rmask, int f32, hipStream_t s,
            int ldx, int acc_dx, bf16_t* dxp, int dx_f32, const float* pre_part, int pre_nparts, float* coef_ext,
            int stage) {
  if (!f32 || acc_dx || (ldx != 0 && ldx != C)) {
    dxp = nullptr;
    dx_f32 = 1;
  }
  if (ldx == 0) ldx = C;
  float* coef = coef_ext ? coef_ext : ws;
  float* part = ws + (long)3 * C * K;
  const int rpb = rows_per_block(R, K);
  dim3 grid(cdiv(R, rpb), K);
  const int V = vw(std::gcd(C, ldx));
  if (V != 8) rmask = nullptr;
  BNCoefArgs ca{gamma, nullptr, mean, rstd, nullptr, nullptr, coef, dgamma, dbeta, dg_cs, g_cs, 0.f, 1, 1};
  DISPATCH_T(f32, {
    if (stage == 2) {
    } else if (pre_part) {
      if (pre_nparts > FOLD && pre_nparts <= cdiv(R, 32)) {
        const int nfold = cdiv(pre_nparts, FOLD);
        double* folds = reinterpret_cast<double*>(ws + bn_fold_offset(K, R, C));
        hipLaunchKernelGGL(part_fold_kernel, dim3(nfold, K), dim3(256), 0, s, pre_part, pre_nparts, 2 * C, folds,
                           nfold);
        launch_coef<TT, double>(dim3(cdiv(C, 32), K), s, (const double*)folds, nfold, CP(gamma), (const TT*)nullptr,
                                valid_rows, mean, rstd, (float*)nullptr, (float*)nullptr, coef, dgamma, dbeta, dg_cs,
                                g_cs, K, R, C, 0.f, 1, 1, 0, 0L);
      } else {
        launch_coef<TT, float>(dim3(cdiv(C, 32), K), s, pre_part, pre_nparts, CP(gamma), (const TT*)nullptr,
                               valid_rows, mean, rstd, (float*)nullptr, (float*)nullptr, coef, dgamma, dbeta, dg_cs,
                               g_cs, K, R, C, 0.f, 1, 1, 0, 0L);
      }
    } else {
      DISPATCH_V(V, hipLaunchKernelGGL((chan_reduce_kernel<TT, VV, 1>), grid, dim3(256), 0, s, CP(dy), CP(x), CP(y),
                                       mean, rstd, valid_rows, R, C, relu, part, (long)2 * C, rpb, rmask, ca, C, ldx));
    }
    if (!pre_part && stage != 2)
      launch_coef<TT, float>(dim3(cdiv(C, 32), K), s, (const float*)part, (int)grid.x, CP(gamma), (const TT*)nullptr,
                             valid_rows, mean, rstd, (float*)nullptr, (float*)nullptr, coef, dgamma, dbeta, dg_cs, g_cs, K,
                             R, C, 0.f, 1, 1, 0, 0L);
    if (stage != 1)
      DISPATCH_V(V, hipLaunchKernelGGL((bn_bwd_apply_kernel<TT, VV>), grid, dim3(256), 0, s, CP(dy), CP(x), CP(y),
                                       valid_rows, coef, R, C, relu, MP(dx), MP(dpre), rpb, rmask, ldx, acc_dx, dxp,
                                       dx_f32));
  });
}

void fold_col_partials(const float* part, int nparts, int C, float* out, long out_cs, int K, hipStream_t s) {
  hipLaunchKernelGGL(part_sum_kernel, dim3(cdiv(C, 256), K), dim3(256), 0, s, part, nparts, C, C, out, (float*)nullptr,
                     out_cs);
}

void bn_bwd_coef_parts(const float* part, int nparts, const float* gamma, long g_cs, const int* valid_rows,
                       const float* mean, const float* rstd, int K, int R, int C, float* coef, float* dgamma,
                       float* dbeta, long dg_cs, hipStream_t s) {
  launch_coef<float, float>(dim3(cdiv(C, 32), K), s, part, nparts, gamma, (const float*)nullptr, valid_rows, mean, rstd,
                            (float*)nullptr, (float*)nullptr, coef, dgamma, dbeta, dg_cs, g_cs, K, R, C, 0.f, 1, 1, 0,
                            0L);
}

void part_sum_f64(const float* part, int K, int nparts, int g, double* out, long out_cs, int ldo, hipStream_t s) {
  if (K == 0) return;
  hipLaunchKernelGGL(part_sum_f64_kernel<float>, dim3(K), dim3(1024), 0, s, part, nparts, g, out, out_cs, ldo);
}

long chan_sums_f64_ws(int R, int C) { return (long)cdiv(R, 256) * 2 * C; }

void chan_sums_f64(const float* x, long x_cs, int ldx, int K, int R, int C, const int* valid, double* ws, double* out,
                   long out_cs, int ldo, hipStream_t s) {
  if (K == 0 || R == 0) return;
  const int rb = 256, nch = cdiv(R, rb);
  hipLaunchKernelGGL(chan_sums_f64_kernel, dim3(nch, K), dim3(256), 0, s, x, x_cs, ldx, R, C, valid, rb, ws, nch);
  hipLaunchKernelGGL(part_sum_f64_kernel<double>, dim3(K), dim3(1024), 0, s, (const double*)ws, nch, C, out, out_cs,
                     ldo);
}

void bn_coef_sums(const double* sums, long sums_cs, int ldp, const float* gamma, const float* beta,
                  const int* valid_rows, long g_cs, int K, int R, int C, float eps, int rep, float* mean, float* rstd,
                  float* coef, hipStream_t s) {
  using TT = float;
  launch_coef<TT, double>(dim3(cdiv(C, 32), K), s, sums, 1, gamma, beta, valid_rows, (const float*)nullptr,
                          (const float*)nullptr, mean, rstd, coef, (float*)nullptr, (float*)nullptr, 0L, g_cs, K, R, C,
                          eps, rep, 0, ldp, sums_cs);
}

long col_sum_workspace_floats(int K, long rows, int C) {
  const int rpb = rows_per_block(rows, K);
  return (long)K * cdiv(rows, rpb) * C;
}

void col_sum(const void* x, float* out, long out_cs, int K, long rows, int C, int f32, hipStream_t s, float* ws) {
  const int rpb = rows_per_block(rows, K);
  dim3 grid(cdiv(rows, rpb), K);
  const int V = vw(C);
  if (ws) {
    DISPATCH_T(f32, DISPATCH_V(V, hipLaunchKernelGGL((chan_reduce_kernel<TT, VV, 3>), grid, dim3(256), 0, s, CP(x),
                                                     nullptr, nullptr, nullptr, nullptr, nullptr, (int)rows, C, 0, ws,
                                                     0L, rpb, nullptr, BNCoefArgs{}, C, C)));
    hipLaunchKernelGGL(part_sum_kernel, dim3(cdiv(C, 256), K), dim3(256), 0, s, ws, (int)grid.x, C, C, out,
// ... 54 lines not shown
```

distributed_learning_simulator_amd/ops/functional.py:

```python

from __future__ import annotations

import collections

import torch

from ..options import OPTIONS
from . import backend, ref
from .fusion import (BNBwdLink, BNOut, BNStats, DeferredBN, DeferredBNBwd, DeferredRes, DeferredStemBN,
                     MaskedGrad, ResidualLink, Tags, _require_fp32, bn_bwd_defer_count,
                     bn_bwd_f32_defer_count, bn_bwd_parts_count, res_fold_count, stem_defer_count, tag, tags)


def _be(t):
    return backend.get(t)


def _given(**kw):
    return {k: v for k, v in kw.items() if v is not None}


def _halo_shape(w, stride, pad) -> bool:
    return stride == 1 and pad == 1 and w.shape[2] == 3 and w.shape[3] == 3


def _stats_part(be, K, rows, C, device):
    return torch.empty((K, be.conv_stats_parts(rows), 2, C), dtype=torch.float32, device=device)


class _Conv(torch.autograd.Function):

    @staticmethod
    def forward(ctx, x, token, w, gw, stride, pad, b, gb, link=None, stats=None, w_split=None, donor=None,
                sgd=None):
        be = _be(x)
        ci = w.shape[-1]
        ctx.sgd = sgd if (sgd is not None and be is not ref and x.dtype == torch.float32 and gw is not None
                          and b is None and x.shape[-1] == ci and w_split is not None) else None
        if x.shape[-1] > ci:
            w = torch.nn.functional.pad(w, (0, x.shape[-1] - ci))
            w_split = None
        if be is ref or x.dtype != torch.float32:
            w_split = None
        tx = tags(x)
        xp = tx.planes
        use_pl = (xp is not None and w_split is not None and x.is_contiguous()
                  and be.conv_planes_ok(x.shape[-1], w.shape[1]) and be.planes_fit(x[0].numel()))
        if tx.planes_only and not use_pl:
            raise RuntimeError("conv2d: planes-only input but the split-plane GEMM cannot run here")
        pl = {"x_planes": xp} if use_pl else {}
        ctx.xp = xp if use_pl else None
        if stats is not None:
            stats.dy_planes_ok = use_pl and b is None
        K, B, H, W = x.shape[:4]
        KH = w.shape[2]
        OH, OW = (H + 2 * pad - KH) // stride + 1, (W + 2 * pad - w.shape[3]) // stride + 1
        y_numel = B * OH * OW * w.shape[1]
        big = be is not ref and max(x[0].numel(), y_numel) * x.element_size() >= (1 << 31)
        if stats is not None:
            stats.dy_planes_ok = stats.dy_planes_ok and be.planes_fit(y_numel)
        want_stats = stats is not None and be is not ref and x.dtype == torch.float32 and not big
        y = None
        ctx.bn_src = None
        defer = tx.bn_defer
        if defer is not None and defer.pending:
            if (OPTIONS.bn_fused_halo and use_pl and _halo_shape(w, stride, pad) and b is None
                    and be.halo_bn_ok(x.shape, w)):
                part = _stats_part(be, K, B * OH * OW, w.shape[1], x.device) if want_stats else None
                bn_wgrad = (defer.write_out and gw is not None and OPTIONS.halo_wgrad
                            and x.shape[-1] == ci and be.halo_wgrad_ok(x.shape, w.shape[1]))
                y = be.conv_halo_bn_fwd(defer.x.view(x.shape), defer.coef, defer.relu, defer.valid_rows, w, w_split,
                                        stats=part, stats_valid=stats.valid if want_stats else None,
                                        yp=defer.yp if defer.write_out and not bn_wgrad else None,
                                        mask=defer.mask if defer.write_out else None)
                if y is not None:
                    defer.taken("conv")
                    if want_stats:
                        stats.part = part
                    if bn_wgrad:
                        ctx.bn_src = (defer.x.view(x.shape), defer.coef, defer.relu, defer.valid_rows)
            defer.materialize()
        if y is None:
            if want_stats:
                stats.part = _stats_part(be, K, B * OH * OW, w.shape[1], x.device)
            st = {"stats": stats.part, "stats_valid": stats.valid} if want_stats else {}
            y = be.conv_fwd(x, w, stride, pad, bias=b, **st, **pl, **_given(w_split=w_split))
        ctx.wgrad_bn_bwd = bool(
            OPTIONS.bn_bwd_in_wgrad_f32 and stats is not None and be is not ref and x.dtype == torch.float32
            and not ctx.needs_input_grad[0] and link is None and donor is None and b is None and gw is not None
            and not use_pl and not big and w.shape[1] % 8 == 0 and x.is_contiguous()
            and be.conv_wgrad_bn_bwd_ok(x.shape, w.shape[1], KH, w.shape[3]))
        if stats is not None:
            stats.wgrad_bn_bwd_ok = ctx.wgrad_bn_bwd
        ctx.w_split = w_split
        ctx.expect_dy_planes = stats is not None and stats.dy_planes_ok
        ctx.x_planes_only = tx.planes_only
        bnb = tx.bnb if OPTIONS.bn_bwd_parts else None
        if bnb is not None and not (be is not ref and donor is None and x.shape[-1] == ci and not big
                                    and be.bn_bwd_parts_ok(x.shape, stride, x.dtype)):
            bnb = None
        ctx.bnb = bnb
        ctx.halo_wgrad = OPTIONS.halo_wgrad
        ctx.valid = stats.valid if (stats is not None and OPTIONS.skip_invalid) else None
        ctx.dgrad_wt = be is not ref
        ctx.save_for_backward(x, w)
        ctx.gw, ctx.gb, ctx.stride, ctx.pad, ctx.ci = gw, gb, stride, pad, ci
        ctx.link = link
        ctx.donor = donor
        if link is not None:
            link.receiver_stride = stride
        return y

    @staticmethod
    def _wgrad(ctx, dy, x, w, dyp, be, bbd=None, sgd_ok=True, bbf=None) -> bool:
        if bbd is not None:
            if not _halo_shape(w, ctx.stride, ctx.pad):
                return False
            sgd = ctx.sgd if sgd_ok else None
            if ctx.bn_src is not None:
                xr, coef, relu, vrows = ctx.bn_src
                ok = be.halo_wgrad(dy, xr, ctx.gw, bn=(coef, relu, vrows), valid=ctx.valid, sgd=sgd,
                                   bn_bwd=bbd.wgrad_args())
            else:
                ok = be.halo_wgrad(dy, x, ctx.gw, x_planes=ctx.xp, valid=ctx.valid, sgd=sgd, bn_bwd=bbd.wgrad_args())
            if ok and sgd is not None:
                sgd[0].done.add(sgd[1])
            return bool(ok)
        padded = w.shape[-1] > ctx.ci
        K = x.shape[0]
        sgd = ctx.sgd if not padded else None
        stepped = False
        gw = torch.empty((K,) + tuple(w.shape[1:]), dtype=torch.float32, device=dy.device) if padded else ctx.gw
        if bbf is not None:
            be.conv_wgrad(dy, x, gw, ctx.stride, ctx.pad, bn_bwd=bbf.wgrad_args())
        elif be is ref:
            gw.copy_(ref.conv_wgrad(dy.float(), x.float(), (K,) + tuple(w.shape[1:]), ctx.stride, ctx.pad))
            if ctx.gb is not None:
                ctx.gb.copy_(dy.float().sum(dim=(1, 2, 3)))
        elif ctx.bn_src is not None:
            xr, coef, relu, vrows = ctx.bn_src
            if not be.halo_wgrad(dy, xr, gw, dy_planes=dyp, bn=(coef, relu, vrows), valid=ctx.valid,
                                 sgd=sgd):
                raise RuntimeError("conv2d backward: the halo wgrad refused a shape its forward accepted")
            stepped = sgd is not None
        elif (ctx.halo_wgrad and _halo_shape(w, ctx.stride, ctx.pad) and not padded
              and be.halo_wgrad(dy, x, gw, dy_planes=dyp, x_planes=ctx.xp, valid=ctx.valid, sgd=sgd)):
            stepped = sgd is not None
        elif dyp is not None:
            stepped = be.conv_wgrad(dy, x, gw, ctx.stride, ctx.pad, dy_planes=dyp, x_planes=ctx.xp, sgd=sgd)
        else:
            if ctx.x_planes_only:
                raise RuntimeError("conv2d backward: fp32 dY with a planes-only input")
# ... 22 lines not shown
                acc = acc.dense()
        acc_compact = False
        if link is not None:
            if acc is not None and link.compact:
                if link.compact == ctx.stride and ctx.stride > 1 and be is not ref and ctx.needs_input_grad[0]:
                    acc_compact = True
                else:
                    full = torch.zeros(x.shape, dtype=acc.dtype, device=acc.device)
                    full[:, :, :: link.compact, :: link.compact] = acc
                    acc = full
            link.grad = None
            link.compact = 0
            if acc is None:
                link.receiver_done = True
        dyp = tags(dy).planes
        wgrad_done = False
        wt_pre = None
        bb = tags(dy).bn_bwd
        if bb is not None and bb.pending and not bb.f32:
            if ctx.gw is not None and be is not ref and ctx.halo_wgrad and w.shape[-1] == ctx.ci:
                sgd_ok = True
                if ctx.sgd is not None and ctx.needs_input_grad[0]:
                    wt_pre = (be.dgrad_wt_prebuild(dy.shape, w, ctx.w_split, x.shape[2:4], ctx.stride, ctx.pad)
                              if ctx.dgrad_wt and ctx.w_split is not None and not acc_compact and ctx.donor is None
                              else None)
                    sgd_ok = wt_pre is not None
                wgrad_done = _Conv._wgrad(ctx, dy, x, w, dyp, be, bb, sgd_ok=sgd_ok)
            if wgrad_done:
                bb.taken("wgrad")
            else:
                bb.materialize()
        elif bb is not None and bb.pending:
            if ctx.wgrad_bn_bwd and not ctx.needs_input_grad[0] and acc is None and dyp is None:
                _Conv._wgrad(ctx, dy, x, w, None, be, bbf=bb)
                wgrad_done = True
                bb.taken("wgrad")
            else:
                bb.materialize()
                tags(dy).planes_only = False
        if dyp is not None and ctx.xp is None:
            raise RuntimeError("conv2d backward: dY planes without the input's planes")
        if dyp is None:
            if ctx.expect_dy_planes:
                raise RuntimeError("conv2d backward: the BN wrote dY as planes only, but they did not arrive")
            if not wgrad_done or ctx.needs_input_grad[0]:
                _require_fp32(dy, "conv2d backward")
        donor = ctx.donor
        compact = (donor is not None and not donor.receiver_done and be is not ref and dy.dtype == torch.float32
                   and ctx.stride > 1 and ctx.pad == 0 and w.shape[2] == 1 and w.shape[3] == 1 and acc is None
                   and w.shape[-1] == ctx.ci and donor.receiver_stride == ctx.stride)
        if ctx.needs_input_grad[0] and compact:
            dx = be.conv_dgrad(dy, w, dy.shape[2:4], 1, 0, w_split=ctx.w_split, **_given(dy_planes=dyp))
        elif ctx.needs_input_grad[0]:
            if acc_compact:
                dx = be.conv_dgrad(dy, w, x.shape[2:4], ctx.stride, ctx.pad, acc=acc, w_split=ctx.w_split,
                                   acc_compact=True, **_given(dy_planes=dyp))
            else:
                bnb = ctx.bnb
                if bnb is not None:
                    K, B, H, W, Ci = x.shape
                    part = _stats_part(be, K, B * H * W, Ci, dy.device)
                dx = be.conv_dgrad(dy, w, x.shape[2:4], ctx.stride, ctx.pad, acc=acc, **_given(
                    bnb=bnb.args(part) if bnb is not None else None, dy_planes=dyp, w_split=ctx.w_split,
                    acc_mask=acc_mask, wt=True if ctx.dgrad_wt else None, wt_buf=wt_pre))
                if bnb is not None:
                    bnb.part, bnb.key = part, (dx.data_ptr(), dx._version)
            if dx.shape[-1] > ctx.ci:
                dx = dx[..., : ctx.ci]
        elif acc is not None:
            dx = acc if acc_mask is None else MaskedGrad(acc, acc_mask).dense()
        if ctx.gw is not None and not wgrad_done:
            _Conv._wgrad(ctx, dy, x, w, dyp, be)
        if donor is not None and dx is not None and not donor.receiver_done:
            donor.grad = dx
            donor.compact = ctx.stride if compact else 0
            dx = None
        return dx, None, None, None, None, None, None, None, None, None, None, None, None


def conv2d(x, token, w, gw, stride=1, pad=0, b=None, gb=None, link: ResidualLink | None = None,
           stats: BNStats | None = None, w_split: torch.Tensor | None = None, donor: ResidualLink | None = None,
           sgd=None):
    if link is not None:
        assert w.shape[-1] == x.shape[-1], "a residual link needs an unpadded conv"
    return _Conv.apply(x, token, w, gw, stride, pad, b, gb, link, stats, w_split, donor, sgd)


class _Linear(torch.autograd.Function):

    @staticmethod
    def forward(ctx, x, token, w, b, gw, gb, residual=None, relu=False, premasked=False, gate_input=False,
                drop_p=0.0, drop_seeds=None, gate_scale=1.0, w_split=None, x_planes=None, out_planes=False,
                dx_planes=False, res_link=None, acc_link=None, sgd=None):
        be = _be(x)
        ctx.res_link, ctx.acc_link = res_link, acc_link
        shp = x.shape
        x = x.reshape(shp[0], -1, shp[-1])
        ctx.res_shape = residual.shape if residual is not None else None
        if residual is not None:
            residual = residual.reshape(shp[0], x.shape[1], -1).contiguous()
        native = be is not ref and x.dtype == torch.float32 and w_split is not None and OPTIONS.planes
        if not native:
            w_split = x_planes = None
            out_planes = dx_planes = False
        if not OPTIONS.tfm_planes:
            out_planes = dx_planes = False
        ws = {"w_split": w_split} if w_split is not None else {}
        xp = {"x_planes": x_planes} if x_planes is not None else {}
        y = be.linear_fwd(x, w, b, relu=relu, acc=residual, drop_p=drop_p, drop_seeds=drop_seeds, **ws, **xp,
                          **({"out_planes": True} if out_planes else {}))
        yp = None
        if out_planes:
            y, yp = y
        ctx.ws = ws
        mask_dy = relu and not premasked
        ctx.save_for_backward(x, w, y if mask_dy else None, drop_seeds if drop_p else None)
        ctx.x_planes = x_planes
        ctx.gw, ctx.gb = gw, gb
        ctx.mask_dy, ctx.gate_input, ctx.has_res = mask_dy, gate_input, residual is not None
# ... 96 lines not shown
    @staticmethod
    def forward(ctx, x, token, w, gw):
        be = _be(x)
        K, Fo, Fi = w.shape
        wcat = w.reshape(1, K * Fo, Fi).contiguous()
        y = be.linear_fwd(x.unsqueeze(0).contiguous(), wcat, None)
        ctx.save_for_backward(x)
        ctx.gw, ctx.K, ctx.Fo = gw, K, Fo
        return y[0].view(-1, K, Fo).permute(1, 0, 2).contiguous()

    @staticmethod
    def backward(ctx, dy):
        (x,) = ctx.saved_tensors
        if ctx.gw is not None:
            be = _be(dy)
            K, Fo = ctx.K, ctx.Fo
            dyc = dy.permute(1, 0, 2).reshape(1, -1, K * Fo).contiguous()
            Fi = x.shape[-1]
            if be is ref:
                dw, _ = ref.linear_wgrad(dyc.float(), x.unsqueeze(0).float(), False)
            else:
                dw = torch.empty((1, K * Fo, Fi), dtype=torch.float32, device=dy.device)
                be.linear_wgrad(dyc, x.unsqueeze(0).contiguous(), dw, None)
            ctx.gw.copy_(dw.view(K, Fo, Fi))
        return None, None, None, None


def linear_shared_input(x, token, w, gw):
    return _LinearSharedInput.apply(x, token, w, gw)


class _BN(torch.autograd.Function):
    @staticmethod
    def forward(ctx, x, token, gamma, beta, ggamma, gbeta, valid_rows, relu, residual, link=None, stats=None,
                planes=BNOut.FP32):
        be = _be(x)
        K = x.shape[0]
        C = x.shape[-1]
        _require_fp32(x, "batch_norm")
        x3 = x.reshape(K, -1, C)
        r3 = res_coef = None
        res_relu = False
        sdef = tags(residual).bn_defer
        if isinstance(sdef, DeferredStemBN):
            if (be is not ref and x.dtype == torch.float32 and sdef.y32 is None and sdef.valid_rows is valid_rows
                    and sdef.x.shape == x3.shape and x3.is_contiguous() and sdef.x.is_contiguous()):
                r3, res_coef, res_relu = sdef.x, sdef.coef, sdef.relu
                stem_defer_count["res"] += 1
            else:
                r3 = sdef.materialize_f32().reshape(K, -1, C)
        elif residual is not None:
            _require_fp32(residual, "batch_norm residual")
            r3 = residual.reshape(K, -1, C)
        mask = yp = bnb = defer = fold_out = None
        fold = tags(residual).res_fold
        if fold is not None and fold.pending:
            if (be is not ref and x.dtype == torch.float32 and fold.valid_rows is valid_rows
                    and fold.x.shape == x3.shape and x3.is_contiguous()):
                r3, res_coef = fold.x, fold.coef
                fold.taken("folded")
            else:
                fold.materialize()
        if be is ref:
            y, mean, rstd = be.bn_fwd(x3, gamma, beta, valid_rows, relu, r3)
        else:
            pre = stats.part if stats is not None else None
            planes = BNOut(planes) if (OPTIONS.planes and x.dtype == torch.float32 and x.is_contiguous()
                                       and be.planes_fit(x[0].numel())) else BNOut.FP32
            wm = any(ctx.needs_input_grad)
            C8 = C % 8 == 0
            can = {BNOut.CONV_DEFER: OPTIONS.bn_fused_halo and C8, BNOut.RES_FOLD: OPTIONS.bn_res_fold and not relu,
                   BNOut.STEM_DEFER: OPTIONS.bn_stem_defer and C8}
            if planes in can and not (can[planes] and residual is None and x3.is_contiguous()):
                planes = planes.applied_now
            if planes is BNOut.RES_FOLD:
                coef, mean, rstd = be.bn_coef(x3, gamma, beta, valid_rows, pre_stats=pre)
                y = torch.empty((K, x3.shape[1], C), dtype=x.dtype, device=x.device)
                fold_out = DeferredRes(x3, coef, valid_rows, y)
            elif planes in (BNOut.CONV_DEFER, BNOut.STEM_DEFER):
                coef, mean, rstd = be.bn_coef(x3, gamma, beta, valid_rows, pre_stats=pre)
                y, yp = be.planes_buffer((K, x3.shape[1], C), x.device)
                mask = torch.empty((K, x3.shape[1], C // 8), dtype=torch.uint8, device=x.device) if (wm and relu) else None
                defer = (DeferredBN if planes is BNOut.CONV_DEFER else DeferredStemBN)(x3, coef, relu, valid_rows, yp,
                                                                                       mask, write_out=wm)
            else:
                out = be.bn_fwd(x3, gamma, beta, valid_rows, relu, r3, with_mask=wm, pre_stats=pre, planes=int(planes),
                                res_coef=res_coef, res_relu=res_relu)
                y, mean, rstd = out[:3]
                mask = out[3] if wm else None
                if planes is not BNOut.FP32:
                    yp = out[-1]
            if stats is not None:
                stats.part = None
            if (wm and OPTIONS.bn_bwd_parts and x.dtype == torch.float32 and x3.is_contiguous()
                    and (mask is not None or not relu)):
                vr = valid_rows.to(torch.int32).contiguous() if valid_rows is not None else None
                bnb = BNBwdLink(x3, mask, mean, rstd, vr)
        ctx.save_for_backward(x3, y if mask is None else None, mean, rstd, gamma)
        ctx.relu_mask = mask
        ctx.valid_rows, ctx.relu, ctx.has_res = valid_rows, relu, residual is not None
        ctx.link = link
        ctx.stats = stats
        ctx.ggamma, ctx.gbeta, ctx.shape = ggamma, gbeta, x.shape
        ctx.bnb = bnb
        ctx.planes_on = OPTIONS.planes
        ctx.bwd_in_wgrad = OPTIONS.bn_bwd_in_wgrad
        ctx.bwd_in_wgrad_f32 = OPTIONS.bn_bwd_in_wgrad_f32
        yo = y.reshape(x.shape)
        if yp is not None:
            tag(yo, planes=yp.view((K, 2) + tuple(x.shape[1:])), planes_only=planes is not BNOut.BOTH)
        ctx.defer = defer
        if defer is not None or fold_out is not None or bnb is not None:
            tag(yo, bn_defer=defer, res_fold=fold_out, bnb=bnb)
        return yo

    @staticmethod
    def backward(ctx, dy):
        x3, y, mean, rstd, gamma = ctx.saved_tensors
        be = _be(dy)
        K, R, C = x3.shape
        if ctx.defer is not None:
            ctx.defer.materialize()
            ctx.defer = None
        dy3 = dy.reshape(K, R, C).contiguous()
        if be is ref:
            dx, dgamma, dbeta, dpre = ref.bn_bwd(dy3, x3, y, mean, rstd, gamma, ctx.valid_rows, ctx.relu)
            if ctx.ggamma is not None:
                ctx.ggamma.copy_(dgamma)
                ctx.gbeta.copy_(dbeta)
        else:
            _require_fp32(dy, "batch_norm backward")
            dxm = 2 if (ctx.stats is not None and ctx.stats.dy_planes_ok and ctx.planes_on) else 0
            pre = None
            bnb = ctx.bnb
            if bnb is not None:
                if bnb.part is not None and bnb.key == (dy3.data_ptr(), dy3._version):
                    pre = bnb.part
                bn_bwd_parts_count["used" if pre is not None else "none" if bnb.part is None else "fallback"] += 1
                bnb.part = bnb.key = None
            masked = (ctx.has_res and ctx.link is not None and ctx.relu and ctx.relu_mask is not None
                      and C % 8 == 0)
            if (dxm == 2 and ctx.bwd_in_wgrad and not (ctx.has_res and not masked) and C % 64 == 0
                    and (ctx.relu_mask is not None or not ctx.relu) and x3.is_contiguous()):
                coef = torch.empty((K, C, 3), dtype=torch.float32, device=dy3.device)
                be.bn_bwd(dy3, x3, y, mean, rstd, gamma, ctx.valid_rows, ctx.relu, ctx.ggamma, ctx.gbeta, False,
                          relu_mask=ctx.relu_mask, pre_part=pre, coef_out=coef)
                dx, dxp = be.planes_buffer((K, R, C), dy3.device)
                if masked:
                    ctx.link.grad = MaskedGrad(dy3.view(ctx.shape), ctx.relu_mask)
                dxo = dx.reshape(ctx.shape)
                tag(dxo, planes=dxp.view((K, 2) + tuple(ctx.shape[1:])), planes_only=True, bn_bwd=DeferredBNBwd(
                    dy3, x3, ctx.relu_mask if ctx.relu else None, coef, ctx.valid_rows, dxp))
                return dxo, None, None, None, None, None, None, None, None, None, None, None
            if (dxm == 0 and ctx.bwd_in_wgrad_f32 and ctx.stats is not None and ctx.stats.wgrad_bn_bwd_ok
                    and not ctx.has_res and C % 8 == 0 and (ctx.relu_mask is not None or not ctx.relu)
                    and x3.is_contiguous() and dy3.dtype == torch.float32):
                coef = torch.empty((K, C, 3), dtype=torch.float32, device=dy3.device)
                be.bn_bwd(dy3, x3, y, mean, rstd, gamma, ctx.valid_rows, ctx.relu, ctx.ggamma, ctx.gbeta, False,
                          relu_mask=ctx.relu_mask, pre_part=pre, coef_out=coef)
                dx = torch.empty((K, R, C), dtype=torch.float32, device=dy3.device)
                dxo = dx.reshape(ctx.shape)
                tag(dxo, planes_only=True, bn_bwd=DeferredBNBwd(
                    dy3, x3, ctx.relu_mask if ctx.relu else None, coef, ctx.valid_rows, dx, f32=True))
                return dxo, None, None, None, None, None, None, None, None, None, None, None
            out = be.bn_bwd(dy3, x3, y, mean, rstd, gamma, ctx.valid_rows, ctx.relu,
                            ctx.ggamma, ctx.gbeta, ctx.has_res and not masked, relu_mask=ctx.relu_mask,
                            dx_planes=dxm, pre_part=pre)
            dx, dpre = out[0], out[1]
            if masked:
                ctx.link.grad = MaskedGrad(dy3.view(ctx.shape), ctx.relu_mask)
            if dxm:
                dxo = dx.reshape(ctx.shape)
                tag(dxo, planes=out[2].view((K, 2) + tuple(ctx.shape[1:])), planes_only=True)
                dres = dpre.reshape(ctx.shape) if (ctx.has_res and not masked) else None
                if dres is not None and ctx.link is not None:
                    ctx.link.grad = dres
                    dres = None
                return dxo, None, None, None, None, None, None, None, dres, None, None, None
            if masked:
                return dx.reshape(ctx.shape), None, None, None, None, None, None, None, None, None, None, None
        dres = dpre.reshape(ctx.shape) if ctx.has_res else None
        if dres is not None and ctx.link is not None:
            ctx.link.grad = dres
            dres = None
        dxo = dx.reshape(ctx.shape)
        if be is not ref:
            tag(dxo, owned=True)
        return dxo, None, None, None, None, None, None, None, dres, None, None, None


def batch_norm(x, token, gamma, beta, ggamma, gbeta, valid_rows=None, relu=False, residual=None,
               link: ResidualLink | None = None, stats: BNStats | None = None, planes: BNOut | int = BNOut.FP32):
    return _BN.apply(x, token, gamma, beta, ggamma, gbeta, valid_rows, relu, residual, link, stats, planes)


class _LN(torch.autograd.Function):
    @staticmethod
    def forward(ctx, x, token, gamma, beta, ggamma, gbeta, planes=False):
        be = _be(x)
        yp = None
        if (planes and OPTIONS.planes and be is not ref and x.dtype == torch.float32
                and be.planes_fit(x[0].numel())):
            y, mean, rstd, yp = be.ln_fwd(x, gamma, beta, planes=True)
        else:
            y, mean, rstd = be.ln_fwd(x, gamma, beta)
        ctx.save_for_backward(x, mean, rstd, gamma)
        ctx.ggamma, ctx.gbeta = ggamma, gbeta
        if yp is not None:
            tag(y, planes=yp)
        return y

    @staticmethod
    def backward(ctx, dy):
        x, mean, rstd, gamma = ctx.saved_tensors
        be = _be(dy)
        dx, dgamma, dbeta = be.ln_bwd(dy.contiguous(), x, mean, rstd, gamma)
        if ctx.ggamma is not None:
            ctx.ggamma.copy_(dgamma)
            ctx.gbeta.copy_(dbeta)
        return dx, None, None, None, None, None, None

# ... 382 lines not shown
```

distributed_learning_simulator_amd/ops/fusion.py:

```python

from __future__ import annotations

import dataclasses
import enum

import torch


class BNOut(enum.IntEnum):

    FP32 = 0
    BOTH = 1
    PLANES = 2
    CONV_DEFER = 3
    RES_FOLD = 4
    STEM_DEFER = 5

    @property
    def applied_now(self) -> "BNOut":
        now = {BNOut.CONV_DEFER: BNOut.PLANES, BNOut.RES_FOLD: BNOut.FP32, BNOut.STEM_DEFER: BNOut.BOTH}
        return now.get(self, self)

    @property
    def reads_planes(self) -> bool:
        return self not in (BNOut.FP32, BNOut.RES_FOLD)


class ResidualLink:

    __slots__ = ("grad", "receiver_done", "compact", "receiver_stride")

    def __init__(self):
        self.grad = None
        self.receiver_done = False
        self.compact = 0
        self.receiver_stride = 1


class MaskedGrad:

    __slots__ = ("dy", "mask")

    def __init__(self, dy, mask):
        self.dy, self.mask = dy, mask

    def dense(self):
        K, C = self.dy.shape[0], self.dy.shape[-1]
        bits = torch.arange(8, device=self.mask.device, dtype=torch.uint8)
        keep = ((self.mask.view(K, -1, C // 8, 1) >> bits) & 1).reshape(K, -1, C).bool()
        return torch.where(keep, self.dy.reshape(K, -1, C), torch.zeros((), dtype=self.dy.dtype,
                                                                          device=self.dy.device)).view(self.dy.shape)


class BNStats:

    __slots__ = ("valid", "part", "dy_planes_ok", "wgrad_bn_bwd_ok")

    def __init__(self, valid=None):
        self.valid = valid
        self.part = None
        self.dy_planes_ok = False
        self.wgrad_bn_bwd_ok = False


bn_bwd_parts_count = {"used": 0, "none": 0, "fallback": 0}


class BNBwdLink:

    __slots__ = ("x", "mask", "mean", "rstd", "valid", "part", "key")

    def __init__(self, x, mask, mean, rstd, valid):
        self.x, self.mask, self.mean, self.rstd, self.valid = x, mask, mean, rstd, valid
        self.part = self.key = None

    def args(self, part):
        return (part, self.x, self.mask, self.mean, self.rstd, self.valid, None)


@dataclasses.dataclass(slots=True, eq=False)
class Tags:

    planes: torch.Tensor | None = None
    planes_only: bool = False
    bn_defer: DeferredBN | None = None
    res_fold: DeferredRes | None = None
    bnb: BNBwdLink | None = None
    bn_bwd: DeferredBNBwd | None = None
    owned: bool = False


class _Untagged(Tags):
    __slots__ = ()

    def __init__(self):
        for f in dataclasses.fields(Tags):
            object.__setattr__(self, f.name, f.default)

    def __setattr__(self, name, value):
        raise AttributeError("the untagged default is shared and read-only: write with tag()")


_UNTAGGED = _Untagged()


def tags(t) -> Tags:
    return getattr(t, "_dls", _UNTAGGED)


def tag(t, record: Tags | None = None, **fields) -> Tags:
    rec = t._dls = record or getattr(t, "_dls", None) or Tags()
    for name, value in fields.items():
        setattr(rec, name, value)
    return rec


def _require_fp32(t, who: str):
    if tags(t).planes_only:
        raise RuntimeError(f"{who}: a planes-only activation reached an op that reads fp32 values")


class Deferral:

    __slots__ = ("pending", "count")

    def __init__(self, count=None):
        self.pending = True
# ... 85 lines not shown
```

distributed_learning_simulator_amd/ops/hip.py:

```python

from __future__ import annotations

import collections
import importlib
import os
import threading

import torch

from ..options import OPTIONS
from . import ref

try:
    _C = importlib.import_module("distributed_learning_simulator_amd._dls_hip")
except ImportError as e:
    raise ImportError(
        "HIP extension _dls_hip is not built; run `python -m distributed_learning_simulator_amd.ops.build` "
        f"(original error: {e})"
    ) from e


def _check_provenance() -> None:
    from . import build as _build

# ... 151 lines not shown

def conv_fwd(x, w, stride: int, pad: int, bias=None, relu=False, out=None, stats=None, stats_valid=None,
             w_split=None, x_planes=None):
    K, B, H, W, C = x.shape
    Kw, Co, KH, KW, Ci = w.shape
    OH, OW = (H + 2 * pad - KH) // stride + 1, (W + 2 * pad - KW) // stride + 1
    per_sample = max(H * W * (x.stride(-2) if x.dim() == 5 else C), OH * OW * Co) * x.element_size()
    if B * per_sample >= WINDOW and stats is None and x_planes is None:
        chunks = _batch_chunks(B, per_sample)
        if out is None:
            out = torch.empty((K, B, OH, OW, Co), dtype=x.dtype, device=x.device)
        for b0, b1 in chunks:
            conv_fwd(x[:, b0:b1], w, stride, pad, bias=bias, relu=relu, out=out[:, b0:b1], w_split=w_split)
        return out
    x, ldx = _pix_stride(x)
    f32 = _f32(x)
    _check(x, x.dtype, contiguous=False, name="x")
    _check(w, x.dtype, contiguous=False, name="w")
    assert Ci == C, (Ci, C)
    w_cs, rep = _client_view(w, K)
    if out is None:
        y, ldy = torch.empty((K, B, OH, OW, Co), dtype=x.dtype, device=x.device), Co
    else:
        assert out.shape == (K, B, OH, OW, Co) and out.dtype == x.dtype
        y, ldy = _pix_stride(out)
        assert y.data_ptr() == out.data_ptr(), "out must be a row-strided view"
    b_cs = 0
    if bias is not None:
        assert bias.dtype == x.dtype
        b_cs, _ = _client_view(bias, K)
    M = B * OH * OW
    if stats is not None:
        assert f32 and stats.dtype == torch.float32 and stats.is_contiguous()
        assert stats.shape == (K, conv_stats_parts(M), 2, Co), stats.shape
    if not f32 and ldx == C and ldy == Co and _gl(K, M, Co, C, KH * KW):
        _C.conv_gl_fwd(_p(x), _p(w), _p(y), _p(bias), B * H * W * C, M * Co, w_cs, b_cs, K, rep, B, H, W, C, OH, OW,
                       KH, KW, stride, pad, Co, int(relu), _s())
        return y
    ws_p, ws_cs, ws_plane = _wsplit_args(w_split if f32 else None, w)
    xp, x_cs, x_lo = _p(x), x.stride(0), 0
    if x_planes is not None and ws_p and planes_ok(C, Co, ldx):
        xp, x_cs, x_lo = _planes_args(x_planes, x)
        planes_launches["fwd"] += 1
    _C.conv_nt(x=xp, w=_p(w), y=_p(y), bias=_p(bias), x_cs=x_cs, y_cs=y.stride(0), w_cs=w_cs, b_cs=b_cs, B=B, H=H, W=W,
               C=C, OH=OH, OW=OW, KH=KH, KW=KW, stride=stride, pad=pad, dil=1, M=M, N=Co, R=KH * KW * Ci, rep=rep,
               relu=int(relu), K=K, variant=nt_f32_variant if f32 else nt_variant, f32=f32, s=_s(), ldx=ldx, ldy=ldy,
               stats=_p(stats), stats_valid=_pi32(stats_valid, K), wsplit=ws_p, ws_cs=ws_cs, ws_plane=ws_plane,
               x_lo=x_lo)
    return y


def bn_bwd_parts_ok(dx_shape, stride: int, dtype) -> bool:
    K, B, H, W, Ci = dx_shape
    return dtype == F32 and stride == 1 and Ci % 4 == 0 and B * H * W * Ci * 4 < WINDOW


def _wt_dgrad_ok(Co, Ci, KH, KW, H, W, stride, pad, planes: bool, ws_p) -> bool:
    return bool(planes and ws_p and stride == 1 and pad == 1 and KH == 3 and KW == 3 and Co % 32 == 0
                and Ci % 32 == 0 and nt_f32_variant < 0 and min(H, W) >= 8)


def dgrad_wt_prebuild(dy_shape, w, w_split, in_hw, stride: int, pad: int):
    K, B, OH, OW, Co = dy_shape
    Kw, Co2, KH, KW, Ci = w.shape
    ws_p, ws_cs, ws_plane = _wsplit_args(w_split, w)
    if not (w.dtype == F32 and planes_ok(Co, Ci, Co)
            and _wt_dgrad_ok(Co, Ci, KH, KW, int(in_hw[0]), int(in_hw[1]), stride, pad, True, ws_p)):
        return None
    wt_buf = torch.empty(Kw * 2 * 9 * Ci * Co, dtype=BF16, device=w.device)
    _C.wt_planes(ws_p, ws_cs, ws_plane, _p(wt_buf), Kw, Co, Ci, _s())
    return wt_buf


def conv_dgrad(dy, w, in_hw, stride: int, pad: int, acc=None, w_split=None, dy_planes=None, acc_compact=False,
               bnb=None, acc_mask=None, wt: bool = False, wt_buf=None):
    K, B, OH, OW, Co = dy.shape
    Kw, Co2, KH, KW, Ci = w.shape
    H, W = int(in_hw[0]), int(in_hw[1])
    per_sample = max(OH * OW * Co, H * W * Ci) * dy.element_size()
    if acc_compact:
        assert stride > 1 and acc is not None and _f32(dy), "compact acc: fp32 strided dgrad only"
        assert acc.shape == (K, B, (H + stride - 1) // stride, (W + stride - 1) // stride, Ci), acc.shape
        assert acc.dtype == dy.dtype and acc.is_contiguous()
    opt = {}
    if bnb is not None:
        part, bx, bmask, bmean, brstd, bvalid, by = bnb
        R = B * H * W
        assert bn_bwd_parts_ok((K, B, H, W, Ci), stride, dy.dtype) and not acc_compact
        assert part.shape == (K, conv_stats_parts(R), 2, Ci) and part.dtype == F32 and part.is_contiguous()
        bx, bxld = _pix_stride(bx.reshape(K, R, -1) if bx.is_contiguous() else bx)
        assert bx.dtype == F32 and bx.shape[-1] == Ci and bx.stride(0) == R * bxld and bxld % 4 == 0
        assert bmean.shape == (K, Ci) and brstd.shape == (K, Ci) and bmean.is_contiguous() and brstd.is_contiguous()
        if bmask is not None:
            assert bmask.dtype == torch.uint8 and bmask.is_contiguous() and bmask.numel() == K * R * Ci // 8
        if by is not None:
            assert by.dtype == F32 and by.is_contiguous() and by.numel() == K * R * Ci
        if bvalid is not None:
            assert bvalid.dtype == torch.int32 and bvalid.shape == (K,) and bvalid.is_contiguous()
        opt["bnb"] = dict(part=_p(part), x=_p(bx), xld=bxld, y=_p(by), mask=_p(bmask), mean=_p(bmean), rstd=_p(brstd),
                          valid=_p(bvalid))
    if acc_mask is not None:
        assert acc is not None and not acc_compact and _f32(dy), "acc_mask: fp32 dgrad with a full-size acc"
        assert acc_mask.dtype == torch.uint8 and acc_mask.is_contiguous() and Ci % 8 == 0
        assert acc_mask.numel() == K * B * H * W * Ci // 8, acc_mask.shape
    if B * per_sample >= WINDOW and dy_planes is None:
        assert bnb is None
        if acc_mask is not None:
            from .fusion import MaskedGrad

            acc, acc_mask = MaskedGrad(acc, acc_mask).dense(), None
        if acc_compact:
            full = torch.zeros((K, B, H, W, Ci), dtype=dy.dtype, device=dy.device)
            full[:, :, ::stride, ::stride] = acc
            acc, acc_compact = full, False
        dx = torch.empty((K, B, H, W, Ci), dtype=dy.dtype, device=dy.device)
        for b0, b1 in _batch_chunks(B, per_sample):
            dx[:, b0:b1] = conv_dgrad(dy[:, b0:b1], w, in_hw, stride, pad,
                                      acc=None if acc is None else acc[:, b0:b1].contiguous(), w_split=w_split)
        return dx
    dy, ld_dy = _pix_stride(dy)
    f32 = _f32(dy)
    _check(w, dy.dtype, contiguous=False, name="w")
    assert Co2 == Co
    w_cs, rep = _client_view(w, K)
    dx = torch.empty((K, B, H, W, Ci), dtype=dy.dtype, device=dy.device)
    if acc is not None and not acc_compact:
        assert acc.shape == dx.shape and acc.dtype == dy.dtype and acc.is_contiguous(), acc.shape
    if (not f32 and not acc_compact and ld_dy == Co and (stride == 1 or (gl_mode == 1 and acc is None))
            and _gl(K, B * H * W, Ci, Co, KH * KW)):
        wt = torch.empty((Kw, Ci, KH, KW, Co), dtype=BF16, device=dy.device)
        _C.conv_weight_flip_t(_p(w), _p(wt), w.stride(0), Kw, Co, KH, KW, Ci, _s())
        _C.conv_gl_dgrad(_p(dy), _p(wt), _p(dx), _p(acc), K, rep, B, OH, OW, Co, H, W, Ci, KH, KW, stride, pad, _s())
        return dx
    ws_p, ws_cs, ws_plane = _wsplit_args(w_split if f32 else None, w)
    dyp, dy_cs, dy_lo = _p(dy), dy.stride(0), 0
    if dy_planes is not None and ws_p and planes_ok(Co, Ci, ld_dy):
        dyp, dy_cs, dy_lo = _planes_args(dy_planes, dy)
        planes_launches["dgrad"] += 1
    wt_ready = wt_buf is not None
    if (wt or wt_ready) and _wt_dgrad_ok(Co, Ci, KH, KW, H, W, stride, pad, bool(dy_lo), ws_p):
        if wt_buf is None:
            wt_buf = torch.empty(Kw * 2 * 9 * Ci * Co, dtype=BF16, device=dy.device)
        planes_launches["dgrad_wt"] += 1
        opt.update(wt_buf=_p(wt_buf), wt_ready=int(wt_ready))
    else:
        assert not wt_ready, "conv_dgrad: a prebuilt wt_buf for a dgrad that does not take it"
    _C.conv_dgrad(dy=dyp, w=_p(w), dx=_p(dx), acc=_p(acc), w_cs=w_cs, K=K, rep=rep, B=B, OH=OH, OW=OW, Co=Co, H=H, W=W,
                  Ci=Ci, KH=KH, KW=KW, stride=stride, pad=pad, variant=nt_f32_variant if f32 else nt_variant, f32=f32,
                  s=_s(), ld_dy=ld_dy, dy_cs=dy_cs, wsplit=ws_p, ws_cs=ws_cs, ws_plane=ws_plane, x_lo=dy_lo,
                  acc_compact=int(bool(acc_compact)), acc_mask=_p(acc_mask), **opt)
    return dx


# ... 483 lines not shown
    if x.dtype != F32 or w.dtype != F32 or w.dim() != 5 or tuple(w.shape[2:]) != (3, 3, C) or C % 4:
        return False
    xs, ldx = _pix_stride(x)
    if xs.data_ptr() != x.data_ptr() or ldx % 8 or x.stride(0) != B * H * W * ldx:
        return False
    return bool(_C.conv_halo_bn_dense_supported(B, H, W, _c32(C), w.shape[1]))


def dense_weight_planes(w) -> torch.Tensor:
    Kw, N, KH, KW, C = w.shape
    C32 = _c32(C)
    assert w.dtype == F32 and w[0].is_contiguous()
    out = torch.empty((Kw, 2, N, KH, KW, C32), dtype=BF16, device=w.device)
    _C.split_rows_padded(_p(w), w.stride(0) if Kw > 1 else 0, Kw, N * KH * KW, C, C32, _p(out), _s())
    return out


def conv_halo_bn_dense_fwd(x, coef, relu: bool, valid_rows, w, out, w_planes=None, stats=None, stats_valid=None,
                           ny=None, mask=None) -> bool:
    K, B, H, W, C = x.shape
    Kw, N = w.shape[0], w.shape[1]
    C32 = _c32(C)
    xs, ldx = _pix_stride(x)
    assert xs.data_ptr() == x.data_ptr(), "x must be a pixel-strided view"
    y, ldy = _pix_stride(out)
    assert y.data_ptr() == out.data_ptr() and out.shape == (K, B, H, W, N), "out must be a pixel-strided view"
    assert coef.shape == (K, C, 2) and coef.dtype == F32
    cp = coef
    if C32 != C:
        cp = torch.zeros((K, C32, 2), dtype=F32, device=x.device)
        cp[:, :C].copy_(coef)
    cp = cp.contiguous()
    if w_planes is None:
        w_planes = dense_weight_planes(w)
    assert w_planes.shape == (Kw, 2, N, 3, 3, C32) and w_planes.dtype == BF16 and w_planes.is_contiguous()
    rep = K // Kw
    if stats is not None:
        assert stats.shape == (K, conv_stats_parts(B * H * W), 2, N) and stats.is_contiguous()
    if ny is not None:
        assert ny.shape == (K, B * H * W, C) and ny.dtype == F32 and ny.is_contiguous()
    if mask is not None:
        assert ny is not None and C % 8 == 0 and mask.shape == (K, B * H * W, C // 8) and mask.dtype == torch.uint8
        assert mask.is_contiguous()
    ok = _C.conv_halo_bn_dense_fwd(
        x=_p(xs), x_cs=xs.stride(0), ldx=ldx, creal=C, coef=_p(cp), relu=int(relu), valid_rows=_pi32(valid_rows),
        wsplit=_p(w_planes), ws_cs=w_planes.stride(0) if Kw > 1 else 0, ws_plane=w_planes.stride(1), rep=rep, y=_p(y),
        y_cs=y.stride(0), ldy=ldy, K=K, B=B, H=H, W=W, C=C32, N=N, stats=_p(stats), stats_valid=_pi32(stats_valid),
        ny=_p(ny), ny_cs=ny.stride(0) if ny is not None else 0, ldny=C, mask=_p(mask), s=_s())
    if ok:
        planes_launches["fwd_bn_dense"] += 1
    return bool(ok)


def bn_bwd(dy, x, y, mean, rstd, gamma, valid_rows, relu, ggamma, gbeta, need_dpre, relu_mask=None, dx_out=None,
           dx_planes: int = 0, pre_part=None, coef_out=None):
    K, R, C = x.shape
    x, ldx = _pix_stride(x)
    assert x.stride(0) == R * ldx
    dy = dy.contiguous()
    g_cs, rep = _client_view(gamma, K)
    assert rep == 1 or gamma.shape[0] == 1, "bn_bwd supports per-client or fully shared γ"
    if dx_out is not None:
        assert dx_out.shape == (K, R, C) and dx_out.stride() == x.stride() and dx_out.dtype == x.dtype
        dx = dx_out
    else:
        assert ldx == C, "strided x needs a strided dx_out"
    dxp = None
    if dx_planes and dx_out is None and x.dtype == F32:
        dx, dxp = _planes_out((K, R, C), x.device, dx_planes)
    else:
        dx_planes = 0
        if dx_out is None:
            dx = torch.empty((K, R, C), dtype=x.dtype, device=x.device)
    dpre = torch.empty((K, R, C), dtype=x.dtype, device=x.device) if need_dpre else None
    ws = _workspace(_C.bn_workspace_floats(K, R, C), x.device)
    dg_cs = ggamma.stride(0) if ggamma is not None else 0
    assert dy.dtype == x.dtype == gamma.dtype
    if pre_part is not None:
        assert pre_part.dtype == F32 and pre_part.is_contiguous() and pre_part.shape == (K, (R + 31) // 32, 2, C)
    if coef_out is not None:
        assert coef_out.shape == (K, C, 3) and coef_out.dtype == F32 and coef_out.is_contiguous()
        assert dx_out is None and not need_dpre
    _C.bn_bwd(dy=_p(dy), x=_p(x), y=_p(y), mean=_p(mean), rstd=_p(rstd), gamma=_p(gamma), valid_rows=_pi32(valid_rows),
              g_cs=g_cs, K=K, R=R, C=C, relu=int(relu), dx=_p(dx), dpre=_p(dpre), dgamma=_p(ggamma), dbeta=_p(gbeta),
              dg_cs=dg_cs, ws=_p(ws), relu_mask=_p(relu_mask), f32=_f32(x), s=_s(), ldx=ldx, dxp=_p(dxp),
              acc_dx=int(dx_out is not None), dx_f32=int(dx_planes != 2), coef_ext=_p(coef_out),
              stage=1 if coef_out is not None else 0, **_pre_part(pre_part, K, C))
    if coef_out is not None:
        return None
    if dx_planes:
        return dx, dpre, dxp
    return dx, dpre


def bn_bwd_apply_planes(dy, x, relu_mask, coef, valid_rows, dxp) -> None:
    K, R, C = x.shape
    assert dxp.shape == (K, 2, R, C) and dxp.is_contiguous()
    _bn_bwd_apply(dy, x, relu_mask, coef, valid_rows, dx=_p(dxp), dxp=_p(dxp), dx_f32=0)


def bn_bwd_apply_f32(dy, x, relu_mask, coef, valid_rows, dx) -> None:
    assert dx.shape == x.shape and dx.dtype == F32 and dx.is_contiguous()
    _bn_bwd_apply(dy, x, relu_mask, coef, valid_rows, dx=_p(dx))


def _bn_bwd_apply(dy, x, relu_mask, coef, valid_rows, **out) -> None:
    K, R, C = x.shape
    assert dy.shape == x.shape and dy.is_contiguous() and x.is_contiguous() and dy.dtype == F32 == x.dtype
    assert coef.shape == (K, C, 3)
    ws = _workspace(_C.bn_workspace_floats(K, R, C), x.device)
    _C.bn_bwd(dy=_p(dy), x=_p(x), valid_rows=_pi32(valid_rows), K=K, R=R, C=C, relu=int(relu_mask is not None),
              ws=_p(ws), relu_mask=_p(relu_mask), f32=1, s=_s(), ldx=C, coef_ext=_p(coef), stage=2, **out)


def ln_fwd(x, gamma, beta, eps=1e-5, planes: bool = False):
    K = x.shape[0]
    C = x.shape[-1]
    x = x.contiguous()
    g_cs, rep = _client_view(gamma, K)
    rpc = x.numel() // (K * C)
    y = torch.empty_like(x)
    mean = torch.empty(x.shape[:-1], dtype=torch.float32, device=x.device)
    rstd = torch.empty_like(mean)
    assert gamma.dtype == x.dtype
    yp = torch.empty((K, 2) + tuple(x.shape[1:]), dtype=BF16, device=x.device) if planes and x.dtype == F32 else None
    _C.ln_fwd(_p(x), _p(gamma), _p(beta), _p(y), _p(mean), _p(rstd), g_cs, K, rpc, C, eps, rep, _f32(x), _s(), _p(yp))
    if planes:
        return y, mean, rstd, yp
    return y, mean, rstd


def ln_bwd(dy, x, mean, rstd, gamma):
    K = x.shape[0]
    C = x.shape[-1]
    assert C <= 1024
    g_cs, rep = _client_view(gamma, K)
    rpc = x.numel() // (K * C)
    dx = torch.empty_like(x)
    if OPTIONS.deterministic:
        dgamma = torch.empty((K, C), dtype=torch.float32, device=x.device)
# ... 837 lines not shown
```

distributed_learning_simulator_amd/options.py:

```python

from __future__ import annotations

import contextlib
import dataclasses
import os
import threading


def _env_bool(name: str, default: bool) -> bool:
    v = os.environ.get(name)
    return default if v is None else v not in ("0", "", "false", "False")


def _env_int(name: str, default: int) -> int:
    v = os.environ.get(name)
    return default if v is None or v == "" else int(v)


@dataclasses.dataclass
class RuntimeOptions:
    planes: bool = dataclasses.field(default_factory=lambda: _env_bool("DLS_PLANES", True))
    """BatchNorms emit bf16 (hi, lo) planes for the LDS-DMA plane / halo GEMMs (off: every conv
    splits its operand in registers)."""
    fused_sgd: bool = dataclasses.field(default_factory=lambda: _env_bool("DLS_FUSED_SGD", True))
    """SGD steps of the weights whose plane / halo wgrad kernels can apply them (csrc/sgd_epi.h)
    run in those kernels; the flat step covers the rest (engine.params.FusedSGD)."""
    tfm_planes: bool = dataclasses.field(default_factory=lambda: _env_bool("DLS_TFM_PLANES", True))
    """Transformer split-plane producers: the FFN hidden activation and its gradient (linear1 /
    linear2 epilogues) and the dropout backward of the residual-branch linears (out_proj /
    linear2) write planes for the plane GEMMs (off: fp32 only). (Attention outputs writing planes
    measured +0.4-0.5 s per FedOBD stage-1 round each, profiles/r5_c6_ab_tfm_planes.txt: removed.)"""
    bn_bwd_parts: bool = dataclasses.field(default_factory=lambda: _env_bool("DLS_BN_BWD_PARTS", True))
    """BN backward partial sums from the consuming conv's dgrad epilogue (off: own reduction)."""
    bn_fused_halo: bool = dataclasses.field(default_factory=lambda: _env_bool("DLS_BN_FUSED_HALO", True))
    """A BN(+ReLU) whose only reader is a 3x3 stride-1 conv (ResNet BasicBlock bn1) is applied in
    that conv's halo loader (ops.fusion DeferredBN; off: BN apply pass + plane conv)."""
    bn_res_fold: bool = dataclasses.field(default_factory=lambda: _env_bool("DLS_BN_RES_FOLD", True))
    """A ResNet downsample shortcut's BN is applied inside the block's last BN apply, which reads
    its raw input as the residual (ops.fusion DeferredRes; off: its own apply pass)."""
    bn_stem_defer: bool = dataclasses.field(default_factory=lambda: _env_bool("DLS_BN_STEM_DEFER", True))
    """The CIFAR ResNet stem BN(+ReLU), read by layer1.0.conv1 (planes) and by layer1.0.bn2 (fp32, as
    its identity residual), is applied by those two readers: the conv in its halo loader, the BN
    in its residual fold (ops.fusion DeferredStemBN; off: one apply pass writes both forms)."""
    dense_bn_halo: bool = dataclasses.field(default_factory=lambda: _env_bool("DLS_DENSE_BN_HALO", True))
    """DenseNet growth convs apply their BN + ReLU in the halo loader over the block buffer's
    channel prefix (off: BN apply pass + implicit-GEMM conv)."""
    halo_wgrad: bool = dataclasses.field(default_factory=lambda: _env_bool("DLS_HALO_WGRAD", True))
    """3x3 stride-1 weight gradients of 64-512-channel convs (ResNet layers 1-3) on the LDS-halo
    kernel (csrc/conv_halo_wgrad.hip; off: the implicit-GEMM TN kernel)."""
    bn_bwd_in_wgrad: bool = dataclasses.field(default_factory=lambda: _env_bool("DLS_BN_BWD_IN_WGRAD", True))
    """A training BN(+ReLU) whose input gradient feeds only a 3x3 stride-1 conv's backward (ResNet
    BasicBlock bn1 / identity-block bn2, layers 1-3) computes its coefficients only: that conv's halo
    weight gradient applies the BN backward in its dY loader and writes dX's planes for the dgrad
    (ops.fusion DeferredBNBwd; off: the BN backward's own apply pass writes them)."""
    bn_bwd_in_wgrad_f32: bool = dataclasses.field(default_factory=lambda: _env_bool("DLS_BN_BWD_IN_WGRAD_F32", True))
    """A training BN(+ReLU) behind a conv whose input needs no gradient (the ResNet stem) computes
    its backward coefficients only: the conv's fp32 weight gradient applies the BN backward in its dY
    loader (ops.fusion DeferredBNBwd f32, csrc/conv_f32.hip; off: the BN backward's own apply pass
    writes dX and the weight gradient reads it back)."""
    dense_wgrad_halo: bool = dataclasses.field(default_factory=lambda: _env_bool("DLS_DENSE_WGRAD_HALO", True))
    """DenseNet growth-conv weight gradients on the LDS-halo kernel (the normalised prefix staged
    once per pixel tile for all nine taps; off: the implicit-GEMM TN kernel)."""
    dense_dgrad_fused: bool = dataclasses.field(default_factory=lambda: _env_bool("DLS_DENSE_DGRAD_FUSED", True))
    """DenseNet growth-conv input gradients fused with the BN backward (csrc/conv_dense_dgrad.hip:
    dX̂ recomputed in a sums pass and an apply pass instead of stored and read twice; off: the
    implicit-GEMM dgrad + the BN backward passes)."""
    dense_y_recompute: bool = dataclasses.field(default_factory=lambda: _env_bool("DLS_DENSE_Y_RECOMPUTE", True))
    """With the fused dgrad and the halo weight gradient, DenseNet training stores no normalised
    activation: both backward kernels rebuild relu(BN(x)) from the raw prefix and the forward's
    (scale, shift), bitwise (off: the forward's halo conv writes it for them)."""
    dense_stats_cache: bool = dataclasses.field(default_factory=lambda: _env_bool("DLS_DENSE_STATS_CACHE", True))
    """DenseNet blocks (fused growth convs) sum each channel's statistics once, from the producing
    conv's epilogue, into running fp64 sums the BN coefficients read (off: a statistics pass over
    the prefix per layer)."""
    deterministic: bool = dataclasses.field(default_factory=lambda: _env_bool("DLS_DETERMINISTIC", True))
    """Split-K weight gradients and column sums folded in a fixed order (off: fp32 atomics)."""
    streams: int = dataclasses.field(default_factory=lambda: _env_int("DLS_STREAMS", 2))
    """Sub-cohort HIP streams trained concurrently on one GPU."""
    ragged_steps: bool = dataclasses.field(default_factory=lambda: _env_bool("DLS_RAGGED_STEPS", True))
    """A cohort's clients are ordered by shard size, so in an epoch's last steps (where only the
    clients with the largest shards still have a batch) the active clients are a row prefix and
    the step runs those rows only (off: every step runs all K rows, idle ones masked)."""
    skip_invalid: bool = dataclasses.field(default_factory=lambda: _env_bool("DLS_SKIP_INVALID", True))
    """Halo convolutions skip the images past a client's valid samples (a partial last batch):
    weight gradients because their dY and X are zeros written by the BatchNorms, forward / dgrad
    tiles whose only readers are BatchNorm passes that stop at the valid rows (off: computed)."""
    graphs: bool = dataclasses.field(default_factory=lambda: _env_bool("DLS_GRAPHS", True))
    """HIP-graph replay of whole training steps (off: eager steps)."""
    max_graphs: int = dataclasses.field(default_factory=lambda: _env_int("DLS_MAX_GRAPHS", 3))
    """Captured step graphs kept per trainer (each owns a private memory pool): a round uses the
    full cohort's and its ragged epoch-end step's (ragged_steps)."""
    eval_max_images: int = dataclasses.field(default_factory=lambda: _env_int("DLS_EVAL_MAX_IMAGES", 4096))
    """Images per evaluation launch (M models x batches): larger launches fill the GPU better and
    cost activation memory; past 4096 they measured slower (GTG utility of 32 models: 38.8 ms per
    model at 4096 vs 39.9 at 8192 and 40.5 at 16384, profiles/r6_c16_eval_max_images.log; the
    headline's one-model test pass equal). Per sub-cohort stream: evaluate() keeps up to `streams` launches in
    flight on separate streams (whose freed blocks the caching allocator does not share), so its
    peak activation memory is about streams x this many images' worth."""
    shared_planes: bool = dataclasses.field(default_factory=lambda: _env_bool("DLS_SHARED_PLANES", True))
    """Shared-model steps (sign-SGD / sync-SGD): every client reads the one shared row's weight
    planes (rep = K) and its activations' planes (off: register-split GEMMs; sign-SGD ResNet-50
    3.51 vs 3.18 s per vote step)."""
    native: dict = dataclasses.field(default_factory=dict)
    """e.g. {"pl_min_wg": 0, "conv_gl": 0, "attn_mfma": 0, "halo_wgrad_unroll": 2}."""


OPTIONS = RuntimeOptions()
_FIELDS = {f.name for f in dataclasses.fields(RuntimeOptions)}


_NATIVE_UNSET = -1000000


def _push_native(native: dict) -> None:
    if not native:
        return
    try:
        from .ops import hip
    except ImportError:
        return
    for k, v in native.items():
        hip._C.set_native_option(str(k), _NATIVE_UNSET if v is None else int(v))


def update(**kw) -> dict:
    old = {}
    for k, v in kw.items():
# ... 69 lines not shown
```

Measured before the change: 0.3018 rounds/s.

## Fuse BN-backward partial sums into stride-2 dgrad and shortcut BN apply

Extends the BN-backward partial-sum fusion to stride-2 dgrad parity-class launches, so the BN before a ResNet downsample block gets its reduction partials from the conv epilogue. The downsample block's last BN apply pass also accumulates the shortcut BN's backward sums while it writes dY. Both changes remove standalone reduction passes over activations. The cost is extra register and shared-memory pressure in the apply kernel, some variant restrictions (variant 10 remapped), and more complex partial-buffer indexing.

```diff
diff --git a/csrc/bindings.cpp b/csrc/bindings.cpp
--- a/csrc/bindings.cpp
+++ b/csrc/bindings.cpp
@@ -131,6 +131,7 @@
     if (b.on()) {
       bnb.part = b.p("part"); bnb.x = b.p("x"); bnb.xld = b.l("xld", 0); bnb.y = b.p("y", 0);
       bnb.mask = b.p("mask", 0); bnb.mean = b.p("mean"); bnb.rstd = b.p("rstd"); bnb.valid = b.p("valid", 0);
+      bnb.nparts = b.i("nparts");
       b.finish();
     }
     a.finish();
@@ -311,10 +312,18 @@
     const int K = a.i("K"), R = a.i("R"), C = a.i("C"), relu = a.i("relu", 0), f32 = a.i("f32");
     const int ldx = a.i("ldx", 0), acc_dx = a.i("acc_dx", 0), dx_f32 = a.i("dx_f32", 1);
     const int pre_nparts = a.i("pre_nparts", 0), stage = a.i("stage", 0);
+    Args c = a.sub("sc");
+    const float *sc_x = nullptr, *sc_mean = nullptr, *sc_rstd = nullptr;
+    float* sc_part = nullptr;
+    if (c.on()) {
+      sc_x = c.p("x"); sc_mean = c.p("mean"); sc_rstd = c.p("rstd"); sc_part = c.p("part");
+      c.finish();
+    }
     a.finish();
     bn_bwd(dy, x, y, mean, rstd, gamma, valid_rows, g_cs, K, R, C, relu, dx, dpre, dgamma, dbeta, dg_cs, ws, relu_mask,
-           f32, s, ldx, acc_dx, dxp, dx_f32, pre_part, pre_nparts, coef_ext, stage);
-  });
+           f32, s, ldx, acc_dx, dxp, dx_f32, pre_part, pre_nparts, coef_ext, stage, sc_x, sc_mean, sc_rstd, sc_part);
+  });
+  m.def("bn_bwd_sc_parts", &bn_bwd_sc_parts);
   m.def("ln_fwd", [](ptr x, ptr gamma, ptr beta, ptr y, ptr mean, ptr rstd, long g_cs, int K, long rpc, int C,
                      float eps, int rep, int f32, ptr s, ptr yp) {
     ln_fwd(P<const void>(x), P<const void>(gamma), P<const void>(beta), P<void>(y), P<float>(mean), P<float>(rstd),
diff --git a/csrc/conv_f32.hip b/csrc/conv_f32.hip
--- a/csrc/conv_f32.hip
+++ b/csrc/conv_f32.hip
@@ -307,7 +307,7 @@
     }
   }
 
-  nt_f32_epilogue<TM, TN, WM * WN, -1, false>(p, acc, smem, client, m0, n0, wm0, wn0, wid, lane);
+  nt_f32_epilogue<TM, TN, WM * WN, -1, false, false, (BKM && BN > 32)>(p, acc, smem, client, m0, n0, wm0, wn0, wid, lane);
 }
 
 template <int BM, int BN, int BK, int WM, int WN, int NBUF, int VSET, int MINW = 1>
@@ -731,6 +731,11 @@
     if (v84 && !(variant == 0 || variant == 3 || variant == 4 || variant == 7 || variant == 10))
       variant = p.N <= 64 ? 4 : 0;
   }
+  if (p.bnb && p.out_s > 1 && variant == 10) variant = v88 ? 9 : 4;
+  if (p.bnb && p.out_s > 1 && !bkm) {
+    fprintf(stderr, "conv_nt_f32: parity-class BN partials need the k-major (dgrad) kernels\n");
+    abort();
+  }
   if (!launch_nt_f32_variant(variant, p, K, va, vb, bkm, s)) fprintf(stderr, "conv_nt_f32: bad variant %d\n", variant);
   if (p.yp) {
     if (p.yp_cs != 2 * p.y_cs || p.yp_lo != p.y_cs || p.ldy != p.N || p.out_s != 1) {
diff --git a/csrc/conv_nt.hip b/csrc/conv_nt.hip
--- a/csrc/conv_nt.hip
+++ b/csrc/conv_nt.hip
@@ -411,10 +411,18 @@
   ConvNTParams p{};
   p.acc_mask = acc_mask;
   if (bnb) {
-    if (!f32 || stride != 1 || Ci % 4 != 0 || (bnb->mask && Ci % 8 != 0) || (bnb->xld && bnb->xld % 4 != 0)) {
-      fprintf(stderr, "conv_dgrad: BN-backward partials need an fp32 stride-1 dgrad with Ci %% 4 == 0\n");
+    int nparts = 0;
+    for (int ph = 0; ph < stride; ++ph)
+      for (int pw = 0; pw < stride; ++pw) {
+        const int Hc = (H - ph + stride - 1) / stride, Wc = (W - pw + stride - 1) / stride;
+        if (Hc > 0 && Wc > 0) nparts += (B * Hc * Wc + 31) / 32;
+      }
+    if (!f32 || Ci % 4 != 0 || (bnb->mask && Ci % 8 != 0) || (bnb->xld && bnb->xld % 4 != 0) || bnb->nparts != nparts) {
+      fprintf(stderr, "conv_dgrad: BN-backward partials need an fp32 dgrad with Ci %% 4 == 0 and %d partial rows\n",
+              nparts);
       abort();
     }
+    p.bnb_npc = nparts;
     p.bnb = bnb->part;
     p.bnb_x = bnb->x;
     p.bnb_xld = bnb->xld ? bnb->xld : Ci;
@@ -484,6 +492,7 @@
     conv_nt(p, K, variant, s);
     return;
   }
+  int bnb_off = 0;
   for (int ph = 0; ph < stride; ++ph) {
     const int Hc = (H - ph + stride - 1) / stride;
     if (Hc <= 0) continue;
@@ -510,6 +519,8 @@
       q.out_pw = pw;
       q.out_H = H;
       q.out_W = W;
+      if (bnb) q.bnb = p.bnb + (long)bnb_off * 2 * Ci;
+      bnb_off += (q.M + 31) / 32;
       if (nkh == 0 || nkw == 0) {
         q.KH = q.KW = 1;
         q.R = 0;
diff --git a/csrc/conv_pl.hip b/csrc/conv_pl.hip
--- a/csrc/conv_pl.hip
+++ b/csrc/conv_pl.hip
@@ -269,7 +269,7 @@
   }
   wait_vm<0>();
 
-  nt_f32_epilogue<TM, TN, NW, -1, true, PIX>(p, acc, smem, client, m0, n0, wm0, wn0, wid, lane);
+  nt_f32_epilogue<TM, TN, NW, -1, true, PIX, !PIX>(p, acc, smem, client, m0, n0, wm0, wn0, wid, lane);
 }
 
 template <int BM, int BN, int WM, int WN, int NST, bool ILV = false, int PKT = 32, int MINW = 1, bool PIX = false>
diff --git a/csrc/dls.h b/csrc/dls.h
--- a/csrc/dls.h
+++ b/csrc/dls.h
@@ -69,6 +69,7 @@
   const float* bnb_mean;
   const float* bnb_rstd;
   const int* bnb_valid;
+  int bnb_npc;
   const float* bn_x;
   long bn_x_cs;
   const float* bn_coef;
@@ -97,6 +98,7 @@
   const float* mean;
   const float* rstd;
   const int* valid;
+  int nparts;
 };
 
 struct DenseWgradParams {
@@ -311,7 +313,10 @@
             const float* pre_part = nullptr,
             int pre_nparts = 0,
             float* coef_ext = nullptr,
-            int stage = 0);
+            int stage = 0,
+            const float* sc_x = nullptr, const float* sc_mean = nullptr, const float* sc_rstd = nullptr,
+            float* sc_part = nullptr);
+int bn_bwd_sc_parts(int K, int R);
 void ln_fwd(const void* x, const void* gamma, const void* beta, void* y, float* mean, float* rstd, long g_cs, int K,
             long rows_per_client, int C, float eps, int rep, int f32, hipStream_t s,
             bf16_t* yp = nullptr);
diff --git a/csrc/epilogue_f32.h b/csrc/epilogue_f32.h
--- a/csrc/epilogue_f32.h
+++ b/csrc/epilogue_f32.h
@@ -2,7 +2,7 @@
 #include "dls.h"
 #include "gemm_common.h"
 
-template <int TM, int TN, int NW, int PF = -1, bool YP = true, bool PIX = false>
+template <int TM, int TN, int NW, int PF = -1, bool YP = true, bool PIX = false, bool SUB = false>
 __device__ __forceinline__ void nt_f32_epilogue(const ConvNTParams& p, f32x16 (&acc)[TM][TN], unsigned char* smem,
                                                 int client, int m0, int n0, int wm0, int wn0, int wid, int lane) {
   constexpr int SW = TN * 32 + 4;
@@ -44,7 +44,8 @@
   static_assert(TN == 1 || TN == 2 || TN == 4 || TN == 8, "column quads per row must divide the wave");
   constexpr int Q = TN * 8;
   const bool bnb = p.bnb != nullptr;
-  const int bnb_rows = bnb ? (p.bnb_valid ? min(p.M, p.bnb_valid[client]) : p.M) : 0;
+  const int xrows = (SUB && p.out_s > 1) ? p.B * p.out_H * p.out_W : p.M;
+  const int bnb_rows = bnb ? (p.bnb_valid ? min(xrows, p.bnb_valid[client]) : xrows) : 0;
   float4 bmu = make_float4(0.f, 0.f, 0.f, 0.f), brs = bmu;
   {
     const int n = n0 + wn0 + (lane % Q) * 4;
@@ -54,8 +55,8 @@
     }
   }
   constexpr int QPL = 4 * TN;
-  const float* bx_base = bnb ? p.bnb_x + (long)client * p.M * p.bnb_xld : nullptr;
-  const unsigned char* bm_base = (bnb && p.bnb_mask) ? p.bnb_mask + (long)client * p.M * (p.N >> 3) : nullptr;
+  const float* bx_base = bnb ? p.bnb_x + (long)client * xrows * p.bnb_xld : nullptr;
+  const unsigned char* bm_base = (bnb && p.bnb_mask) ? p.bnb_mask + (long)client * xrows * (p.N >> 3) : nullptr;
   const float* by_base = (bnb && p.bnb_y) ? p.bnb_y + (long)client * p.y_cs : nullptr;
   auto ld4 = [](const float* base, long off, bool ok) {
     const float4 v = *reinterpret_cast<const float4*>(ok ? base + off : base);
@@ -78,6 +79,10 @@
   auto vrow = [&](int m) -> long {
     if constexpr (PIX) return row_of(m);
     return m;
+  };
+  auto brow = [&](int m, long row) -> long {
+    if constexpr (SUB) return row;
+    return vrow(m);
   };
   __syncthreads();
 #pragma unroll
@@ -120,10 +125,10 @@
         if (accp) av[t % NS] = ld4(accp, (p.acc_compact ? (long)m : row) * p.ldy + n, ok);
         if (amask) amv[t % NS] = abits(row, n, ok);
         if (bnb) {
-          const bool okb = ok && vrow(m) < bnb_rows;
+          const bool okb = ok && brow(m, row) < bnb_rows;
           xv[t % NS] = ld4(bx_base, row * p.bnb_xld + n, okb);
           if (bm_base) {
-            const uint32_t mb = *(okb ? bm_base + vrow(m) * (p.N >> 3) + (n >> 3) : bm_base);
+            const uint32_t mb = *(okb ? bm_base + brow(m, row) * (p.N >> 3) + (n >> 3) : bm_base);
             mv[t % NS] = okb ? (mb >> (n & 4)) : 0u;
           } else if (by_base) {
             const float4 yv = ld4(by_base, row * p.ldy + n, okb);
@@ -252,12 +257,12 @@
           }
           *reinterpret_cast<float4*>(dst) = v;
           if (YP && ypl) store_pl4(row * p.ldy + n, v);
-          if (bnb && vrow(m) < bnb_rows) {
+          if (bnb && (int)brow(m, row) < bnb_rows) {
             const float4 xv =
-                *reinterpret_cast<const float4*>(p.bnb_x + ((long)client * p.M + row) * p.bnb_xld + n);
+                *reinterpret_cast<const float4*>(p.bnb_x + ((long)client * xrows + row) * p.bnb_xld + n);
             uint32_t mb = 0xFu;
             if (p.bnb_mask) {
-              mb = p.bnb_mask[((long)client * p.M + vrow(m)) * (p.N >> 3) + (n >> 3)] >> (n & 4);
+              mb = p.bnb_mask[((long)client * xrows + brow(m, row)) * (p.N >> 3) + (n >> 3)] >> (n & 4);
             } else if (p.bnb_y) {
               const float4 yv = *reinterpret_cast<const float4*>(p.bnb_y + (long)client * p.y_cs + row * p.ldy + n);
               mb = (yv.x > 0.f ? 1u : 0u) | (yv.y > 0.f ? 2u : 0u) | (yv.z > 0.f ? 4u : 0u) | (yv.w > 0.f ? 8u : 0u);
@@ -298,7 +303,8 @@
       }
       const int g0 = m0 + wm0 + i * 32, n = n0 + wn0 + lane * 4;
       if (lane < Q && g0 < p.M && n < p.N) {
-        float* part = p.bnb + ((long)client * ((p.M + 31) / 32) + g0 / 32) * 2 * p.N;
+        const int npc = (SUB && p.out_s > 1) ? p.bnb_npc : (p.M + 31) / 32;
+        float* part = p.bnb + ((long)client * npc + g0 / 32) * 2 * p.N;
         *reinterpret_cast<float4*>(part + n) = bs0;
         *reinterpret_cast<float4*>(part + p.N + n) = bs1;
       }
diff --git a/csrc/norm.hip b/csrc/norm.hip
--- a/csrc/norm.hip
+++ b/csrc/norm.hip
@@ -416,14 +416,22 @@
   }
 }
 
-template <typename T, int V>
+struct BNShortcutSums {
+  const float* x;
+  const float* mean;
+  const float* rstd;
+  float* part;
+};
+
+template <typename T, int V, bool SC = false>
 __global__ void __launch_bounds__(256) bn_bwd_apply_kernel(const T* __restrict__ dy, const T* __restrict__ x,
                                                            const T* __restrict__ y,
                                                            const int* __restrict__ valid_rows,
                                                            const float* __restrict__ coef, int R, int C, int relu,
                                                            T* __restrict__ dx, T* __restrict__ dpre,
                                                            int rpb, const uint8_t* __restrict__ rmask, int ldx,
-                                                           int acc_dx, bf16_t* __restrict__ dxp, int dx_f32) {
+                                                           int acc_dx, bf16_t* __restrict__ dxp, int dx_f32,
+                                                           BNShortcutSums sc) {
   const int k = blockIdx.y;
   const int CT = C / V;
   const int nvalid = valid_rows ? min(valid_rows[k], R) : R;
@@ -433,8 +441,9 @@
     const int ctn = min(256, CT - cg);
     const int RT = 256 / ctn;
     const int cc = threadIdx.x % ctn, rl = threadIdx.x / ctn;
-    if (rl >= RT) continue;
-    const int c0 = (cg + cc) * V;
+    if (!SC && rl >= RT) continue;
+    const bool active = rl < RT;
+    const int c0 = active ? (cg + cc) * V : 0;
     float ca[V], cd[V], ce[V];
 #pragma unroll
     for (int j = 0; j < V; ++j) {
@@ -443,7 +452,16 @@
       cd[j] = coef[q + 1];
       ce[j] = coef[q + 2];
     }
-    for (int r = r0 + rl; r < r1; r += RT) {
+    float s0[SC ? V : 1], s1[SC ? V : 1], smu[SC ? V : 1], srs[SC ? V : 1];
+    if constexpr (SC) {
+#pragma unroll
+      for (int j = 0; j < V; ++j) {
+        s0[j] = s1[j] = 0.f;
+        smu[j] = sc.mean[(long)k * C + c0 + j];
+        srs[j] = sc.rstd[(long)k * C + c0 + j];
+      }
+    }
+    for (int r = r0 + rl; r < (active ? r1 : 0); r += RT) {
       const long off = base + (long)r * C + c0;
       const long offx = base_x + (long)r * ldx + c0;
       float o[V], gp[V];
@@ -451,6 +469,8 @@
         float vdy[V], vx[V];
         load_vec<V>(dy + off, vdy);
         load_vec<V>(x + offx, vx);
+        float vsx[SC ? V : 1];
+        if constexpr (SC) load_vec<V>(sc.x + off, vsx);
         if (rmask) {
           const uint32_t mbits = rmask[((long)k * R + r) * (C / 8) + c0 / 8];
 #pragma unroll
@@ -466,6 +486,13 @@
           gp[j] = vdy[j];
           o[j] = fmaf(ca[j], vdy[j], fmaf(ce[j], vx[j], cd[j]));
         }
+        if constexpr (SC) {
+#pragma unroll
+          for (int j = 0; j < V; ++j) {
+            s0[j] += gp[j];
+            s1[j] += gp[j] * (vsx[j] - smu[j]) * srs[j];
+          }
+        }
       } else {
 #pragma unroll
         for (int j = 0; j < V; ++j) o[j] = gp[j] = 0.f;
@@ -482,6 +509,32 @@
         store_planes<V>(hp, hp + (long)R * C, o);
       }
       if (dpre) store_vec<V>(dpre + off, gp);
+    }
+    if constexpr (SC) {
+      __shared__ float red[2][256 * V];
+#pragma unroll
+      for (int j = 0; j < V; ++j) {
+        red[0][threadIdx.x * V + j] = s0[j];
+        red[1][threadIdx.x * V + j] = s1[j];
+      }
+      __syncthreads();
+      if (active && rl == 0) {
+        for (int t = 1; t < RT; ++t) {
+          const int t2 = t * ctn + cc;
+#pragma unroll
+          for (int j = 0; j < V; ++j) {
+            s0[j] += red[0][t2 * V + j];
+            s1[j] += red[1][t2 * V + j];
+          }
+        }
+        float* part = sc.part + ((long)k * gridDim.x + blockIdx.x) * 2 * C;
+#pragma unroll
+        for (int j = 0; j < V; ++j) {
+          part[c0 + j] = s0[j];
+          part[C + c0 + j] = s1[j];
+        }
+      }
+      __syncthreads();
     }
   }
 }
@@ -696,13 +749,15 @@
 #define CP(p) static_cast<const TT*>(p)
 #define MP(p) static_cast<TT*>(p)
 
+static int pre_parts_max(long R) { return cdiv((int)R, 32) + 3; }
+
 static long bn_fold_offset(int K, long R, int C) {
   const long parts = (R + rows_per_block(R, K) - 1) / rows_per_block(R, K);
   return ((long)K * 3 * C + (long)K * parts * 2 * C + 1) & ~1L;
 }
 
 long bn_workspace_floats(int K, long R, int C) {
-  const long nfold = cdiv((int)cdiv((int)R, 32), FOLD);
+  const long nfold = cdiv(pre_parts_max(R), FOLD);
   return bn_fold_offset(K, R, C) + (long)K * nfold * 2 * C * 2;
 }
 
@@ -764,7 +819,7 @@
             const int* valid_rows, long g_cs, int K, int R, int C, int relu, void* dx, void* dpre, float* dgamma,
             float* dbeta, long dg_cs, float* ws, const uint8_t* rmask, int f32, hipStream_t s,
             int ldx, int acc_dx, bf16_t* dxp, int dx_f32, const float* pre_part, int pre_nparts, float* coef_ext,
-            int stage) {
+            int stage, const float* sc_x, const float* sc_mean, const float* sc_rstd, float* sc_part) {
   if (!f32 || acc_dx || (ldx != 0 && ldx != C)) {
     dxp = nullptr;
     dx_f32 = 1;
@@ -780,7 +835,7 @@
   DISPATCH_T(f32, {
     if (stage == 2) {
     } else if (pre_part) {
-      if (pre_nparts > FOLD && pre_nparts <= cdiv(R, 32)) {
+      if (pre_nparts > FOLD && pre_nparts <= pre_parts_max(R)) {
         const int nfold = cdiv(pre_nparts, FOLD);
         double* folds = reinterpret_cast<double*>(ws + bn_fold_offset(K, R, C));
         hipLaunchKernelGGL(part_fold_kernel, dim3(nfold, K), dim3(256), 0, s, pre_part, pre_nparts, 2 * C, folds,
@@ -801,12 +856,24 @@
       launch_coef<TT, float>(dim3(cdiv(C, 32), K), s, (const float*)part, (int)grid.x, CP(gamma), (const TT*)nullptr,
                              valid_rows, mean, rstd, (float*)nullptr, (float*)nullptr, coef, dgamma, dbeta, dg_cs, g_cs, K,
                              R, C, 0.f, 1, 1, 0, 0L);
-    if (stage != 1)
+    const BNShortcutSums sc{sc_x, sc_mean, sc_rstd, sc_part};
+    if (sc_part) {
+      if (!f32 || V != 8 || !dpre || stage == 1 || !sc_x || !sc_mean || !sc_rstd) {
+        fprintf(stderr, "bn_bwd: the shortcut BN's sums need an fp32 apply pass with dpre and C %% 8 == 0\n");
+        abort();
+      }
+      hipLaunchKernelGGL((bn_bwd_apply_kernel<float, 8, true>), grid, dim3(256), 0, s, (const float*)dy,
+                         (const float*)x, (const float*)y, valid_rows, coef, R, C, relu, (float*)dx, (float*)dpre, rpb,
+                         rmask, ldx, acc_dx, dxp, dx_f32, sc);
+    } else if (stage != 1) {
       DISPATCH_V(V, hipLaunchKernelGGL((bn_bwd_apply_kernel<TT, VV>), grid, dim3(256), 0, s, CP(dy), CP(x), CP(y),
                                        valid_rows, coef, R, C, relu, MP(dx), MP(dpre), rpb, rmask, ldx, acc_dx, dxp,
-                                       dx_f32));
+                                       dx_f32, sc));
+    }
   });
 }
+
+int bn_bwd_sc_parts(int K, int R) { return cdiv(R, rows_per_block(R, K)); }
 
 void fold_col_partials(const float* part, int nparts, int C, float* out, long out_cs, int K, hipStream_t s) {
   hipLaunchKernelGGL(part_sum_kernel, dim3(cdiv(C, 256), K), dim3(256), 0, s, part, nparts, C, C, out, (float*)nullptr,
diff --git a/distributed_learning_simulator_amd/ops/functional.py b/distributed_learning_simulator_amd/ops/functional.py
--- a/distributed_learning_simulator_amd/ops/functional.py
+++ b/distributed_learning_simulator_amd/ops/functional.py
@@ -9,7 +9,8 @@
 from . import backend, ref
 from .fusion import (BNBwdLink, BNOut, BNStats, DeferredBN, DeferredBNBwd, DeferredRes, DeferredStemBN,
                      MaskedGrad, ResidualLink, Tags, _require_fp32, bn_bwd_defer_count,
-                     bn_bwd_f32_defer_count, bn_bwd_parts_count, res_fold_count, stem_defer_count, tag, tags)
+                     bn_bwd_f32_defer_count, bn_bwd_parts_count, bn_bwd_parts_strided_count, bn_bwd_sc_sums_count,
+                     res_fold_count, stem_defer_count, tag, tags)
 
 
 def _be(t):
@@ -97,7 +98,8 @@
         ctx.x_planes_only = tx.planes_only
         bnb = tx.bnb if OPTIONS.bn_bwd_parts else None
         if bnb is not None and not (be is not ref and donor is None and x.shape[-1] == ci and not big
-                                    and be.bn_bwd_parts_ok(x.shape, stride, x.dtype)):
+                                    and be.bn_bwd_parts_ok(x.shape, stride, x.dtype)
+                                    and (stride == 1 or OPTIONS.bn_bwd_parts_strided)):
             bnb = None
         ctx.bnb = bnb
         ctx.halo_wgrad = OPTIONS.halo_wgrad
@@ -226,19 +228,21 @@
         if ctx.needs_input_grad[0] and compact:
             dx = be.conv_dgrad(dy, w, dy.shape[2:4], 1, 0, w_split=ctx.w_split, **_given(dy_planes=dyp))
         elif ctx.needs_input_grad[0]:
+            bnb = ctx.bnb
+            if bnb is not None:
+                K, B, H, W, Ci = x.shape
+                part = torch.empty((K, be.bn_bwd_parts_rows(B, H, W, ctx.stride), 2, Ci), dtype=torch.float32,
+                                   device=dy.device)
             if acc_compact:
                 dx = be.conv_dgrad(dy, w, x.shape[2:4], ctx.stride, ctx.pad, acc=acc, w_split=ctx.w_split,
-                                   acc_compact=True, **_given(dy_planes=dyp))
-            else:
-                bnb = ctx.bnb
-                if bnb is not None:
-                    K, B, H, W, Ci = x.shape
-                    part = _stats_part(be, K, B * H * W, Ci, dy.device)
+                                   acc_compact=True, **_given(dy_planes=dyp,
+                                                              bnb=bnb.args(part) if bnb is not None else None))
+            else:
                 dx = be.conv_dgrad(dy, w, x.shape[2:4], ctx.stride, ctx.pad, acc=acc, **_given(
                     bnb=bnb.args(part) if bnb is not None else None, dy_planes=dyp, w_split=ctx.w_split,
                     acc_mask=acc_mask, wt=True if ctx.dgrad_wt else None, wt_buf=wt_pre))
-                if bnb is not None:
-                    bnb.part, bnb.key = part, (dx.data_ptr(), dx._version)
+            if bnb is not None:
+                bnb.fill(part, dx, "strided" if ctx.stride > 1 else "dgrad")
             if dx.shape[-1] > ctx.ci:
                 dx = dx[..., : ctx.ci]
         elif acc is not None:
@@ -441,13 +445,14 @@
         elif residual is not None:
             _require_fp32(residual, "batch_norm residual")
             r3 = residual.reshape(K, -1, C)
-        mask = yp = bnb = defer = fold_out = None
+        mask = yp = bnb = defer = fold_out = sc_link = None
         fold = tags(residual).res_fold
         if fold is not None and fold.pending:
             if (be is not ref and x.dtype == torch.float32 and fold.valid_rows is valid_rows
                     and fold.x.shape == x3.shape and x3.is_contiguous()):
                 r3, res_coef = fold.x, fold.coef
                 fold.taken("folded")
+                sc_link = tags(residual).bnb if (OPTIONS.bn_bwd_parts and OPTIONS.bn_bwd_sc_sums) else None
             else:
                 fold.materialize()
         if be is ref:
@@ -492,6 +497,8 @@
         ctx.stats = stats
         ctx.ggamma, ctx.gbeta, ctx.shape = ggamma, gbeta, x.shape
         ctx.bnb = bnb
+        ctx.sc_link = sc_link if (sc_link is not None and sc_link.mask is None and C % 8 == 0
+                                  and sc_link.x.shape == x3.shape) else None
         ctx.planes_on = OPTIONS.planes
         ctx.bwd_in_wgrad = OPTIONS.bn_bwd_in_wgrad
         ctx.bwd_in_wgrad_f32 = OPTIONS.bn_bwd_in_wgrad_f32
@@ -523,10 +530,13 @@
             pre = None
             bnb = ctx.bnb
             if bnb is not None:
-                if bnb.part is not None and bnb.key == (dy3.data_ptr(), dy3._version):
-                    pre = bnb.part
-                bn_bwd_parts_count["used" if pre is not None else "none" if bnb.part is None else "fallback"] += 1
-                bnb.part = bnb.key = None
+                pre, source = bnb.take(dy3)
+                hit = "used" if pre is not None else "fallback"
+                if source in (None, "dgrad"):
+                    bn_bwd_parts_count[hit if source else "none"] += 1
+                else:
+                    bn_bwd_parts_count["none"] += 1
+                    (bn_bwd_parts_strided_count if source == "strided" else bn_bwd_sc_sums_count)[hit] += 1
             masked = (ctx.has_res and ctx.link is not None and ctx.relu and ctx.relu_mask is not None
                       and C % 8 == 0)
             if (dxm == 2 and ctx.bwd_in_wgrad and not (ctx.has_res and not masked) and C % 64 == 0
@@ -552,10 +562,16 @@
                 tag(dxo, planes_only=True, bn_bwd=DeferredBNBwd(
                     dy3, x3, ctx.relu_mask if ctx.relu else None, coef, ctx.valid_rows, dx, f32=True))
                 return dxo, None, None, None, None, None, None, None, None, None, None, None
+            sc = ctx.sc_link if (ctx.has_res and not masked and x3.is_contiguous()) else None
+            if sc is not None:
+                sc_part = torch.empty((K, be.bn_bwd_sc_parts(K, R), 2, C), dtype=torch.float32, device=dy3.device)
             out = be.bn_bwd(dy3, x3, y, mean, rstd, gamma, ctx.valid_rows, ctx.relu,
                             ctx.ggamma, ctx.gbeta, ctx.has_res and not masked, relu_mask=ctx.relu_mask,
-                            dx_planes=dxm, pre_part=pre)
+                            dx_planes=dxm, pre_part=pre,
+                            **_given(sc=(sc.x, sc.mean, sc.rstd, sc_part) if sc is not None else None))
             dx, dpre = out[0], out[1]
+            if sc is not None:
+                sc.fill(sc_part, dpre, "sc")
             if masked:
                 ctx.link.grad = MaskedGrad(dy3.view(ctx.shape), ctx.relu_mask)
             if dxm:
diff --git a/distributed_learning_simulator_amd/ops/fusion.py b/distributed_learning_simulator_amd/ops/fusion.py
--- a/distributed_learning_simulator_amd/ops/fusion.py
+++ b/distributed_learning_simulator_amd/ops/fusion.py
@@ -64,15 +64,28 @@
 
 
 bn_bwd_parts_count = {"used": 0, "none": 0, "fallback": 0}
+bn_bwd_parts_strided_count = {"used": 0, "fallback": 0}
+bn_bwd_sc_sums_count = {"used": 0, "fallback": 0}
 
 
 class BNBwdLink:
 
-    __slots__ = ("x", "mask", "mean", "rstd", "valid", "part", "key")
+    __slots__ = ("x", "mask", "mean", "rstd", "valid", "part", "key", "source")
 
     def __init__(self, x, mask, mean, rstd, valid):
         self.x, self.mask, self.mean, self.rstd, self.valid = x, mask, mean, rstd, valid
         self.part = self.key = None
+        self.source = None
+
+    def fill(self, part, dy, source):
+        self.part, self.key, self.source = part, (dy.data_ptr(), dy._version), source
+
+    def take(self, dy):
+        part, source = self.part, self.source
+        if part is not None and self.key != (dy.data_ptr(), dy._version):
+            part = None
+        self.part = self.key = self.source = None
+        return part, source
 
     def args(self, part):
         return (part, self.x, self.mask, self.mean, self.rstd, self.valid, None)
diff --git a/distributed_learning_simulator_amd/ops/hip.py b/distributed_learning_simulator_amd/ops/hip.py
--- a/distributed_learning_simulator_amd/ops/hip.py
+++ b/distributed_learning_simulator_amd/ops/hip.py
@@ -227,7 +227,12 @@
 
 def bn_bwd_parts_ok(dx_shape, stride: int, dtype) -> bool:
     K, B, H, W, Ci = dx_shape
-    return dtype == F32 and stride == 1 and Ci % 4 == 0 and B * H * W * Ci * 4 < WINDOW
+    return dtype == F32 and stride in (1, 2) and Ci % 4 == 0 and B * H * W * Ci * 4 < WINDOW
+
+
+def bn_bwd_parts_rows(B: int, H: int, W: int, stride: int = 1) -> int:
+    return sum(conv_stats_parts(B * len(range(ph, H, stride)) * len(range(pw, W, stride)))
+               for ph in range(min(stride, H)) for pw in range(min(stride, W)))
 
 
 def _wt_dgrad_ok(Co, Ci, KH, KW, H, W, stride, pad, planes: bool, ws_p) -> bool:
@@ -261,8 +266,9 @@
     if bnb is not None:
         part, bx, bmask, bmean, brstd, bvalid, by = bnb
         R = B * H * W
-        assert bn_bwd_parts_ok((K, B, H, W, Ci), stride, dy.dtype) and not acc_compact
-        assert part.shape == (K, conv_stats_parts(R), 2, Ci) and part.dtype == F32 and part.is_contiguous()
+        assert bn_bwd_parts_ok((K, B, H, W, Ci), stride, dy.dtype) and not (acc_compact and stride == 1)
+        assert part.shape == (K, bn_bwd_parts_rows(B, H, W, stride), 2, Ci), part.shape
+        assert part.dtype == F32 and part.is_contiguous()
         bx, bxld = _pix_stride(bx.reshape(K, R, -1) if bx.is_contiguous() else bx)
         assert bx.dtype == F32 and bx.shape[-1] == Ci and bx.stride(0) == R * bxld and bxld % 4 == 0
         assert bmean.shape == (K, Ci) and brstd.shape == (K, Ci) and bmean.is_contiguous() and brstd.is_contiguous()
@@ -273,7 +279,7 @@
         if bvalid is not None:
             assert bvalid.dtype == torch.int32 and bvalid.shape == (K,) and bvalid.is_contiguous()
         opt["bnb"] = dict(part=_p(part), x=_p(bx), xld=bxld, y=_p(by), mask=_p(bmask), mean=_p(bmean), rstd=_p(brstd),
-                          valid=_p(bvalid))
+                          valid=_p(bvalid), nparts=part.shape[1])
     if acc_mask is not None:
         assert acc is not None and not acc_compact and _f32(dy), "acc_mask: fp32 dgrad with a full-size acc"
         assert acc_mask.dtype == torch.uint8 and acc_mask.is_contiguous() and Ci % 8 == 0
@@ -863,11 +869,23 @@
     return bool(ok)
 
 
+def bn_bwd_sc_parts(K: int, R: int) -> int:
+    return _C.bn_bwd_sc_parts(K, R)
+
+
 def bn_bwd(dy, x, y, mean, rstd, gamma, valid_rows, relu, ggamma, gbeta, need_dpre, relu_mask=None, dx_out=None,
-           dx_planes: int = 0, pre_part=None, coef_out=None):
+           dx_planes: int = 0, pre_part=None, coef_out=None, sc=None):
     K, R, C = x.shape
     x, ldx = _pix_stride(x)
     assert x.stride(0) == R * ldx
+    opt = {}
+    if sc is not None:
+        sx, smean, srstd, spart = sc
+        assert need_dpre and coef_out is None and x.dtype == F32 and C % 8 == 0 and ldx == C
+        assert sx.shape == (K, R, C) and sx.dtype == F32 and sx.is_contiguous()
+        assert smean.shape == (K, C) and srstd.shape == (K, C) and smean.is_contiguous() and srstd.is_contiguous()
+        assert spart.shape == (K, bn_bwd_sc_parts(K, R), 2, C) and spart.dtype == F32 and spart.is_contiguous()
+        opt["sc"] = dict(x=_p(sx), mean=_p(smean), rstd=_p(srstd), part=_p(spart))
     dy = dy.contiguous()
     g_cs, rep = _client_view(gamma, K)
     assert rep == 1 or gamma.shape[0] == 1, "bn_bwd supports per-client or fully shared γ"
@@ -888,7 +906,7 @@
     dg_cs = ggamma.stride(0) if ggamma is not None else 0
     assert dy.dtype == x.dtype == gamma.dtype
     if pre_part is not None:
-        assert pre_part.dtype == F32 and pre_part.is_contiguous() and pre_part.shape == (K, (R + 31) // 32, 2, C)
+        assert pre_part.dim() == 4 and pre_part.shape[1] >= 1, pre_part.shape
     if coef_out is not None:
         assert coef_out.shape == (K, C, 3) and coef_out.dtype == F32 and coef_out.is_contiguous()
         assert dx_out is None and not need_dpre
@@ -896,7 +914,7 @@
               g_cs=g_cs, K=K, R=R, C=C, relu=int(relu), dx=_p(dx), dpre=_p(dpre), dgamma=_p(ggamma), dbeta=_p(gbeta),
               dg_cs=dg_cs, ws=_p(ws), relu_mask=_p(relu_mask), f32=_f32(x), s=_s(), ldx=ldx, dxp=_p(dxp),
               acc_dx=int(dx_out is not None), dx_f32=int(dx_planes != 2), coef_ext=_p(coef_out),
-              stage=1 if coef_out is not None else 0, **_pre_part(pre_part, K, C))
+              stage=1 if coef_out is not None else 0, **_pre_part(pre_part, K, C), **opt)
     if coef_out is not None:
         return None
     if dx_planes:
diff --git a/distributed_learning_simulator_amd/options.py b/distributed_learning_simulator_amd/options.py
--- a/distributed_learning_simulator_amd/options.py
+++ b/distributed_learning_simulator_amd/options.py
@@ -32,6 +32,10 @@
     measured +0.4-0.5 s per FedOBD stage-1 round each, profiles/r5_c6_ab_tfm_planes.txt: removed.)"""
     bn_bwd_parts: bool = dataclasses.field(default_factory=lambda: _env_bool("DLS_BN_BWD_PARTS", True))
     """BN backward partial sums from the consuming conv's dgrad epilogue (off: own reduction)."""
+    bn_bwd_parts_strided: bool = dataclasses.field(
+        default_factory=lambda: _env_bool("DLS_BN_BWD_PARTS_STRIDED", True))
+    """... also from a stride-2 dgrad's parity-class launches (the last BN before a ResNet downsample
+    block; off, or bn_bwd_parts off: that BN's own reduction pass)."""
     bn_fused_halo: bool = dataclasses.field(default_factory=lambda: _env_bool("DLS_BN_FUSED_HALO", True))
     """A BN(+ReLU) whose only reader is a 3x3 stride-1 conv (ResNet BasicBlock bn1) is applied in
     that conv's halo loader (ops.fusion DeferredBN; off: BN apply pass + plane conv)."""
@@ -73,6 +77,9 @@
     """DenseNet blocks (fused growth convs) sum each channel's statistics once, from the producing
     conv's epilogue, into running fp64 sums the BN coefficients read (off: a statistics pass over
     the prefix per layer)."""
+    bn_bwd_sc_sums: bool = dataclasses.field(default_factory=lambda: _env_bool("DLS_BN_BWD_SC_SUMS", True))
+    """A ResNet downsample block's last BN sums the shortcut BN's backward partials while its apply
+    pass writes that BN's dY (off, or bn_bwd_parts off: the shortcut BN's own reduction pass)."""
     deterministic: bool = dataclasses.field(default_factory=lambda: _env_bool("DLS_DETERMINISTIC", True))
     """Split-K weight gradients and column sums folded in a fixed order (off: fp32 atomics)."""
     streams: int = dataclasses.field(default_factory=lambda: _env_int("DLS_STREAMS", 2))
```

After: 0.3022 rounds/s, median of 2. Within noise of the previous version (+0.1%).
